# wenxiaoshuai/Points-Matching

Hardware: AMD Instinct MI355X
Metric: descriptor-pair distances/s (BF-L2 2-NN + ratio stage); RANSAC hypotheses/s in `ransac` (higher is better)
Workload: dtype f32

## Files before the change

include/pm.h:

```cpp
#ifndef PM_H_
#define PM_H_

#include <stddef.h>
#include <stdint.h>

#ifdef __cplusplus
extern "C" {
#endif

#define PM_VERSION_MAJOR 0
#define PM_VERSION_MINOR 1

typedef enum pm_status {
    PM_OK            =  0,
    PM_E_INVALID     = -1,
    PM_E_TOO_FEW     = -2,
    PM_E_NO_MODEL    = -3,
    PM_E_HIP         = -4,
    PM_E_NOMEM       = -5,
    PM_E_UNSUPPORTED = -6
} pm_status;

typedef struct pm_match {
    int32_t queryIdx;
    int32_t trainIdx;
    int32_t imgIdx;
    float   distance;
} pm_match;

typedef struct pm_ctx pm_ctx;

int  pm_ctx_create(int device, pm_ctx** out);
int  pm_ctx_destroy(pm_ctx* ctx);
int  pm_ctx_set_stream(pm_ctx* ctx, void* hip_stream);
int  pm_ctx_synchronize(pm_ctx* ctx);
int  pm_ctx_timing_enable(pm_ctx* ctx, int enable);
int  pm_ctx_timing_reset(pm_ctx* ctx);
int  pm_ctx_timing_get(pm_ctx* ctx, const char* kernel, double* mean_ms, int* launches);
int  pm_ctx_knn_diag_enable(pm_ctx* ctx, int enable);
int  pm_ctx_knn_stats(pm_ctx* ctx, int* rescans, int* nonfinite);
int  pm_ctx_knn_route(pm_ctx* ctx, int* route);
int  pm_ctx_filter_fusion_status(pm_ctx* ctx, int* gave_up);
enum {
    PM_OPT_RANSAC_PATH    = 1,
    PM_OPT_SCORE_OPERANDS = 2,
    PM_OPT_HAMMING_ROUTE  = 3,
    PM_OPT_KNN_F16_WAVES  = 4,
    PM_OPT_KNN_STAGING    = 6,
    PM_OPT_KNN_WG_PER_CU  = 7,
    PM_OPT_FILTER_FUSION  = 5,
    PM_OPT_KNN_XCD_TILE   = 8,
    PM_OPT_KNN_GENERAL_F16 = 9,
    PM_OPT_KNN_SEEDED     = 10,
    PM_OPT_KNN_U8_GROUP   = 11,
    PM_OPT_KNN_RING       = 12,
    PM_OPT_KNN_U8_REFINE  = 13,
    PM_OPT_KNN_RING_PROLOGUE = 14,
    PM_OPT_KNN_WIDE       = 15,
    PM_OPT_KNN_PREP_ROWS  = 16,
    PM_OPT_RANSAC_FORM    = 17,
    PM_OPT_RANSAC_WG_IDS  = 18,
    PM_OPT_HAMMING_REFINE = 19,
    PM_OPT_COUNT_         = 20
};
int  pm_ctx_set_option(pm_ctx* ctx, int option, int value);
int  pm_ctx_get_option(pm_ctx* ctx, int option, int* value);
const char* pm_last_error(void);
const char* pm_status_string(int status);
int  pm_version(void);

#define PM_MAX_K 16
#define PM_KNN_FORCE_EXACT  1
#define PM_KNN_FORCE_F32    2
#define PM_KNN_HINT_INTEGER 4
#define PM_KNN_HINT_U8      8
#define PM_KNN_HINT_UNIT_NORM 16
int pm_bf_knn_l2_f32(pm_ctx* ctx, const float* q, int nq, const float* t, int nt,
                     int dim, int k, int flags, pm_match* out);
int pm_bf_knn_l2_f32_dev(pm_ctx* ctx, const float* d_q, int nq, const float* d_t, int nt,
                         int dim, int k, int flags, pm_match* d_out);

int pm_bf_knn_l2_u8(pm_ctx* ctx, const uint8_t* q, int nq, const uint8_t* t, int nt, int dim, int k, pm_match* out);
int pm_bf_knn_l2_u8_dev(pm_ctx* ctx, const uint8_t* d_q, int nq, const uint8_t* d_t, int nt, int dim, int k, pm_match* d_out);
int pm_bf_knn_l2_u8_ratio_dev(pm_ctx* ctx, const uint8_t* d_q, int nq, const uint8_t* d_t, int nt, int dim, float ratio,
                              const float* d_kp1_xy, const float* d_kp2_xy, pm_match* d_knn, pm_match* d_good,
                              float* d_xy1, float* d_xy2, int32_t* d_n_good);

int pm_bf_knn_l2_ratio_dev(pm_ctx* ctx, const float* d_q, int nq, const float* d_t, int nt, int dim, int flags,
                           float ratio, const float* d_kp1_xy, const float* d_kp2_xy, pm_match* d_knn,
                           pm_match* d_good, float* d_xy1, float* d_xy2, int32_t* d_n_good);

typedef struct pm_flann_params {
    int32_t  trees;
    int32_t  checks;
    uint64_t seed;
} pm_flann_params;
typedef struct pm_flann_index pm_flann_index;
int pm_flann_build(pm_ctx* ctx, const float* train, int nt, int dim, const pm_flann_params* prm, pm_flann_index** out);
int pm_flann_destroy(pm_flann_index* ix);
int pm_flann_knn_l2_f32(pm_ctx* ctx, pm_flann_index* ix, const float* q, int nq, int k, pm_match* out);
int pm_flann_knn_l2_f32_dev(pm_ctx* ctx, pm_flann_index* ix, const float* d_q, int nq, int k, pm_match* d_out);
int pm_flann_export(const pm_flann_index* ix, int32_t* n_nodes, int32_t* roots, void* nodes, int32_t cap_nodes);

int pm_bf_knn_hamming_u8(pm_ctx* ctx, const uint8_t* q, int nq, const uint8_t* t, int nt,
                         int bytes, int k, pm_match* out);
int pm_bf_knn_hamming_u8_dev(pm_ctx* ctx, const uint8_t* d_q, int nq, const uint8_t* d_t, int nt,
                             int bytes, int k, pm_match* d_out);


int pm_filter_midpoint(const pm_match* m, int n, double* min_out, double* max_out,
                       pm_match* out, int* n_out);
int pm_filter_ratio(const pm_match* knn, int nq, int k, float ratio, pm_match* out, int* n_out);
int pm_filter_ratio_gather_dev(pm_ctx* ctx, const pm_match* d_knn, int nq, int k, float ratio,
                               const float* d_kp1_xy, const float* d_kp2_xy, pm_match* d_good,
                               float* d_xy1, float* d_xy2, int32_t* d_n_good);
int pm_filter_midpoint_gather_dev(pm_ctx* ctx, const pm_match* d_m, int n, int k,
                                  const float* d_kp1_xy, const float* d_kp2_xy, pm_match* d_good,
                                  float* d_xy1, float* d_xy2, int32_t* d_n_good, double* d_minmax);
int pm_concat_points_dev(pm_ctx* ctx, const float* d_xy1_parts, const float* d_xy2_parts,
                         const int32_t* d_counts, int parts, int stride, float* d_xy1,
                         float* d_xy2, int32_t* d_n_total);

int pm_match_indices(const pm_match* m, int n, int32_t* query_idx, int32_t* train_idx);
int pm_gather_points(const float* kp_xy, int n_kp, const int32_t* idx, int n, float* out_xy);
long pm_format_match_list(const pm_match* m, int n, char* buf, size_t cap);

enum { PM_ERR_SAMPSON = 0, PM_ERR_SYM_EPIPOLAR = 1 };

typedef struct pm_ransac_params {
    int64_t  hyp_begin;
    int64_t  hyp_end;
    uint64_t seed;
    float    thresh_px;
    int32_t  error_kind;
} pm_ransac_params;

int pm_ransac_fundamental(pm_ctx* ctx, const float* xy1, const float* xy2, int n,
                          const pm_ransac_params* p, double F[9], uint8_t* mask,
                          int* n_inliers, uint64_t* best_key);
int pm_ransac_score_dev(pm_ctx* ctx, const float* d_xy1, const float* d_xy2, int n,
                        const pm_ransac_params* p, uint64_t* d_best_key);
int pm_ransac_score_devn(pm_ctx* ctx, const float* d_xy1, const float* d_xy2, int n_max,
                         const int32_t* d_n, const pm_ransac_params* p, uint64_t* d_best_key);
int pm_ransac_run_dev(pm_ctx* ctx, const float* d_xy1, const float* d_xy2, int n_max,
                      const int32_t* d_n, const pm_ransac_params* p, uint64_t* d_best_key,
                      double* d_F, uint8_t* d_mask, int32_t* d_n_inliers);
int pm_ransac_model_from_key_dev(pm_ctx* ctx, const float* d_xy1, const float* d_xy2, int n_max,
                                 const int32_t* d_n, const pm_ransac_params* p,
                                 const uint64_t* d_key, double* d_F, uint8_t* d_mask,
                                 int32_t* d_n_inliers);
int pm_ransac_model_from_hyp(pm_ctx* ctx, const float* xy1, const float* xy2, int n,
                             const pm_ransac_params* p, int64_t hyp, double F[9],
                             uint8_t* mask, int* n_inliers);
#define PM_MAX_PARTS 64
typedef struct pm_points_view {
    const float*   xy1;
    const float*   xy2;
    const int32_t* counts;
    int32_t parts;
    int32_t cap;
    int64_t pitch_xy;
    int32_t pitch_cnt;
    int32_t reserved;
} pm_points_view;
typedef struct pm_ransac_record {
    uint64_t key;
    double   F[9];
} pm_ransac_record;
int pm_ransac_shard_parts_dev(pm_ctx* ctx, const pm_points_view* view, const pm_ransac_params* p,
                              pm_ransac_record* d_record);
int pm_ransac_finish_parts_dev(pm_ctx* ctx, const pm_points_view* view, const pm_ransac_params* p,
                               const pm_ransac_record* d_records, int n_records, uint64_t* d_key, double* d_F,
                               uint8_t* d_mask, int mask_len, int32_t* d_n_inliers, int32_t* d_n_total);
static inline uint64_t pm_ransac_key(uint32_t inliers, uint32_t hyp) {
    return ((uint64_t)inliers << 32) | (uint64_t)(0xFFFFFFFFu - hyp);
}
static inline uint32_t pm_ransac_key_hyp(uint64_t key)     { return 0xFFFFFFFFu - (uint32_t)key; }
static inline uint32_t pm_ransac_key_inliers(uint64_t key) { return (uint32_t)(key >> 32); }

enum { PM_ERR_REPROJ = 2 };
int pm_ransac_homography(pm_ctx* ctx, const float* xy1, const float* xy2, int n, const pm_ransac_params* p,
                         double H[9], uint8_t* mask, int* n_inliers, uint64_t* best_key);
int pm_ransac_homography_run_dev(pm_ctx* ctx, const pm_points_view* view, const pm_ransac_params* p,
                                 uint64_t* d_best_key, double* d_H, uint8_t* d_mask, int mask_len,
                                 int32_t* d_n_inliers);
int pm_ransac_homography_from_hyp(pm_ctx* ctx, const float* xy1, const float* xy2, int n,
                                  const pm_ransac_params* p, int64_t hyp, double H[9], uint8_t* mask,
                                  int* n_inliers);

typedef struct pm_h_refine_info {
    double  cost_in, cost_out;
    int32_t n_used, iters, status, reserved;
} pm_h_refine_info;
int pm_homography_refine(pm_ctx* ctx, const float* xy1, const float* xy2, int n, const uint8_t* mask,
                         const double H_in[9], int max_iters, double H_out[9], pm_h_refine_info* info);
int pm_homography_refine_dev(pm_ctx* ctx, const pm_points_view* view, const uint8_t* d_mask, const double* d_H_in,
                             int max_iters, double* d_H_out, pm_h_refine_info* d_info);
int pm_ransac_homography_refined(pm_ctx* ctx, const float* xy1, const float* xy2, int n, const pm_ransac_params* p,
                                 int max_iters, double H[9], uint8_t* mask, int* n_inliers, uint64_t* best_key,
                                 pm_h_refine_info* info);

enum { PM_AFFINE_FULL = 0, PM_AFFINE_PARTIAL = 1 };
int pm_ransac_affine(pm_ctx* ctx, int model, const float* xy1, const float* xy2, int n, const pm_ransac_params* p,
                     double A[6], uint8_t* mask, int* n_inliers, uint64_t* best_key);
int pm_ransac_affine_from_hyp(pm_ctx* ctx, int model, const float* xy1, const float* xy2, int n,
                              const pm_ransac_params* p, int64_t hyp, double A[6], uint8_t* mask, int* n_inliers);
int pm_ransac_affine_run_dev(pm_ctx* ctx, int model, const pm_points_view* view, const pm_ransac_params* p,
                             uint64_t* d_best_key, double* d_A, uint8_t* d_mask, int mask_len, int32_t* d_n_inliers);
int pm_affine_refine(pm_ctx* ctx, int model, const float* xy1, const float* xy2, int n, const uint8_t* mask,
                     const double A_in[6], double A_out[6], pm_h_refine_info* info);
int pm_affine_refine_dev(pm_ctx* ctx, int model, const pm_points_view* view, const uint8_t* d_mask, const double* d_A_in,
                         double* d_A_out, pm_h_refine_info* d_info);
int pm_estimate_affine(pm_ctx* ctx, int model, const float* xy1, const float* xy2, int n, const pm_ransac_params* p,
                       int refine, double A[6], uint8_t* mask, int* n_inliers, uint64_t* best_key,
                       pm_h_refine_info* info);

// ... 101 lines not shown
```

points_matching_amd/api.py:

```python
import ctypes as C
import os

import numpy as np

_HERE = os.path.dirname(os.path.abspath(__file__))
LIB_PATH = os.environ.get("PM_LIB_PATH") or os.path.join(_HERE, "libpm_hip.so")

MATCH_DTYPE = np.dtype([("queryIdx", "<i4"), ("trainIdx", "<i4"), ("imgIdx", "<i4"),
                        ("distance", "<f4")])
PM_MAX_K = 16
PM_KNN_FORCE_EXACT = 1
PM_KNN_FORCE_F32 = 2
PM_KNN_HINT_INTEGER = 4
PM_KNN_HINT_U8 = 8
PM_KNN_HINT_UNIT_NORM = 16
PM_ERR_SAMPSON = 0
PM_ERR_SYM_EPIPOLAR = 1
PM_ERR_REPROJ = 2
PM_AFFINE_FULL = 0
PM_AFFINE_PARTIAL = 1
PM_OK, PM_E_INVALID, PM_E_TOO_FEW, PM_E_NO_MODEL, PM_E_HIP, PM_E_NOMEM, PM_E_UNSUPPORTED = \
    0, -1, -2, -3, -4, -5, -6

EXPORTS = [
    "pm_ctx_create", "pm_ctx_destroy", "pm_ctx_set_stream", "pm_ctx_synchronize",
    "pm_ctx_timing_enable", "pm_ctx_timing_reset", "pm_ctx_timing_get", "pm_ctx_knn_diag_enable", "pm_ctx_knn_stats", "pm_ctx_knn_route",
    "pm_ctx_filter_fusion_status",
    "pm_last_error",
    "pm_status_string", "pm_version",
    "pm_bf_knn_l2_f32", "pm_bf_knn_l2_f32_dev", "pm_bf_knn_hamming_u8", "pm_bf_knn_hamming_u8_dev",
    "pm_filter_midpoint", "pm_filter_ratio", "pm_match_indices", "pm_gather_points",
    "pm_format_match_list",
    "pm_filter_ratio_gather_dev", "pm_filter_midpoint_gather_dev", "pm_concat_points_dev",
    "pm_ransac_fundamental", "pm_ransac_score_dev", "pm_ransac_score_devn", "pm_ransac_model_from_hyp",
    "pm_ransac_model_from_key_dev", "pm_ransac_run_dev", "pm_ransac_shard_parts_dev", "pm_ransac_finish_parts_dev",
    "pm_ctx_set_option", "pm_ctx_get_option", "pm_bf_knn_l2_ratio_dev",
    "pm_flann_build", "pm_flann_destroy", "pm_flann_knn_l2_f32", "pm_flann_knn_l2_f32_dev", "pm_flann_export",
    "pm_mgpu_create", "pm_mgpu_destroy", "pm_mgpu_size", "pm_mgpu_ctx", "pm_mgpu_ransac_fundamental", "pm_mgpu_match_ransac",
    "pm_mgpu_lane_ctx", "pm_mgpu_set_lanes", "pm_mgpu_set_train", "pm_mgpu_set_train_dev", "pm_mgpu_submit_dev", "pm_mgpu_collect",
    "pm_mgpu_allgather_latency", "pm_mgpu_batch_run", "pm_mgpu_batch_set_option",
    "pm_batch_create", "pm_batch_destroy", "pm_batch_run", "pm_batch_set_option", "pm_batch_set_desc_type", "pm_batch_set_host_threads",
    "pm_bf_knn_l2_u8", "pm_bf_knn_l2_u8_dev", "pm_bf_knn_l2_u8_ratio_dev", "pm_host_register", "pm_host_unregister",
    "pm_lmeds_fundamental", "pm_lmeds_fundamental_dev", "pm_lmeds_default_iters", "pm_ransac7_adaptive",
    "pm_epipolar_residuals", "pm_f_scale_f33", "pm_epilines", "pm_epiline_endpoints",
    "pm_ransac_homography", "pm_ransac_homography_run_dev", "pm_ransac_homography_from_hyp",
    "pm_homography_refine", "pm_homography_refine_dev", "pm_ransac_homography_refined",
    "pm_ransac_affine", "pm_ransac_affine_from_hyp", "pm_ransac_affine_run_dev", "pm_affine_refine", "pm_affine_refine_dev",
    "pm_estimate_affine",
    "pm_ransac_essential", "pm_ransac_essential_from_hyp", "pm_ransac_essential_run_dev", "pm_recover_pose",
    "pm_recover_pose_dev", "pm_estimate_pose",
]


class PmError(RuntimeError):
    def __init__(self, status, msg):
        super().__init__("pm status %d: %s" % (status, msg))
        self.status = status


class RansacParams(C.Structure):
    _fields_ = [("hyp_begin", C.c_int64), ("hyp_end", C.c_int64), ("seed", C.c_uint64),
                ("thresh_px", C.c_float), ("error_kind", C.c_int32)]


class PointsView(C.Structure):
    _fields_ = [("xy1", C.c_void_p), ("xy2", C.c_void_p), ("counts", C.c_void_p), ("parts", C.c_int32),
                ("cap", C.c_int32), ("pitch_xy", C.c_int64), ("pitch_cnt", C.c_int32), ("reserved", C.c_int32)]


class Camera(C.Structure):
    _fields_ = [("fx", C.c_double), ("fy", C.c_double), ("cx", C.c_double), ("cy", C.c_double)]


def _camera(K):
    if isinstance(K, Camera):
        return K
    k = np.asarray(K, np.float64)
    if k.shape == (3, 3):
        return Camera(k[0, 0], k[1, 1], k[0, 2], k[1, 2])
    return Camera(*[float(v) for v in k.reshape(4)])


class HRefineInfo(C.Structure):
    _fields_ = [("cost_in", C.c_double), ("cost_out", C.c_double), ("n_used", C.c_int32), ("iters", C.c_int32),
                ("status", C.c_int32), ("reserved", C.c_int32)]


H_REFINE_INFO_DTYPE = np.dtype([("cost_in", "<f8"), ("cost_out", "<f8"), ("n_used", "<i4"), ("iters", "<i4"),
                                ("status", "<i4"), ("reserved", "<i4")])

RANSAC_RECORD_DTYPE = np.dtype([("key", "<u8"), ("F", "<f8", (9,))])
PM_MAX_PARTS = 64
PM_OPT_RANSAC_PATH, PM_OPT_SCORE_OPERANDS, PM_OPT_HAMMING_ROUTE, PM_OPT_KNN_F16_WAVES, PM_OPT_FILTER_FUSION = 1, 2, 3, 4, 5
PM_OPT_KNN_STAGING = 6
PM_OPT_KNN_WG_PER_CU = 7
PM_OPT_KNN_XCD_TILE = 8
PM_OPT_KNN_GENERAL_F16 = 9
PM_OPT_KNN_SEEDED = 10
PM_OPT_KNN_U8_GROUP = 11
PM_OPT_KNN_RING = 12
PM_OPT_KNN_U8_REFINE = 13
PM_OPT_KNN_RING_PROLOGUE = 14
PM_OPT_KNN_WIDE = 15
PM_OPT_KNN_PREP_ROWS = 16
PM_OPT_RANSAC_FORM = 17
PM_OPT_RANSAC_WG_IDS = 18
PM_OPT_HAMMING_REFINE = 19


_lib = None


def lib():
    global _lib
    if _lib is None:
        if not os.path.exists(LIB_PATH):
            raise PmError(PM_E_UNSUPPORTED,
                          "%s is missing: run `python -m points_matching_amd.build`" % LIB_PATH)
        try:
            import torch
        except ImportError:
            pass
        _lib = C.CDLL(LIB_PATH)
        _lib.pm_last_error.restype = C.c_char_p
        _lib.pm_status_string.restype = C.c_char_p
        _lib.pm_format_match_list.restype = C.c_long
    return _lib


def _check(rc):
    if rc != PM_OK:
        raise PmError(rc, (lib().pm_last_error() or b"").decode() or
                      lib().pm_status_string(rc).decode())


def _p(a):
    return a.ctypes.data_as(C.c_void_p) if a is not None else None


def _pair(xy1, xy2):
    xy1 = np.ascontiguousarray(xy1, np.float32).reshape(-1, 2)
    xy2 = np.ascontiguousarray(xy2, np.float32).reshape(-1, 2)
    if xy2.shape[0] != xy1.shape[0]:
        raise ValueError("xy1 and xy2 must have the same length")
    return xy1, xy2, xy1.shape[0]


def _outcome(rc):
    if rc not in (PM_OK, PM_E_NO_MODEL, PM_E_TOO_FEW):
        _check(rc)
    return rc


def ransac_key(inliers, hyp):
    return (int(inliers) << 32) | (0xFFFFFFFF - int(hyp))


def ransac_key_hyp(key):
    return 0xFFFFFFFF - (int(key) & 0xFFFFFFFF)


def ransac_key_inliers(key):
    return int(key) >> 32



def filter_midpoint(m):
    m = np.ascontiguousarray(m, MATCH_DTYPE).reshape(-1)
    out = np.zeros(max(m.size, 1), MATCH_DTYPE)
    mn, mx, n = C.c_double(), C.c_double(), C.c_int()
    _check(lib().pm_filter_midpoint(_p(m), m.size, C.byref(mn), C.byref(mx), _p(out), C.byref(n)))
    return out[:n.value].copy(), mn.value, mx.value


def filter_ratio(knn, ratio):
    knn = np.ascontiguousarray(knn, MATCH_DTYPE)
    nq, k = knn.shape
    out = np.zeros(max(nq, 1), MATCH_DTYPE)
    n = C.c_int()
    _check(lib().pm_filter_ratio(_p(knn), nq, k, C.c_float(ratio), _p(out), C.byref(n)))
    return out[:n.value].copy()


def match_indices(m):
    m = np.ascontiguousarray(m, MATCH_DTYPE).reshape(-1)
    qi = np.zeros(m.size, np.int32)
    ti = np.zeros(m.size, np.int32)
    _check(lib().pm_match_indices(_p(m), m.size, _p(qi), _p(ti)))
    return qi, ti


def gather_points(kp_xy, idx):
    kp_xy = np.ascontiguousarray(kp_xy, np.float32).reshape(-1, 2)
    idx = np.ascontiguousarray(idx, np.int32)
    out = np.zeros((idx.size, 2), np.float32)
    _check(lib().pm_gather_points(_p(kp_xy), kp_xy.shape[0], _p(idx), idx.size, _p(out)))
    return out


def format_match_list(m):
    m = np.ascontiguousarray(m, MATCH_DTYPE).reshape(-1)
    need = lib().pm_format_match_list(_p(m), m.size, None, C.c_size_t(0))
    buf = C.create_string_buffer(need + 1)
    lib().pm_format_match_list(_p(m), m.size, buf, C.c_size_t(need + 1))
    return buf.value.decode()


def epipolar_residuals(xy1, xy2, F, transposed=1):
    xy1 = np.ascontiguousarray(xy1, np.float32)
    xy2 = np.ascontiguousarray(xy2, np.float32)
    F = np.ascontiguousarray(F, np.float64).reshape(9)
    n = xy1.shape[0]
    r = np.zeros(max(n, 1), np.float64)
    mean = C.c_double()
    _check(lib().pm_epipolar_residuals(_p(xy1), _p(xy2), n, _p(F), transposed, _p(r), C.byref(mean)))
    return r[:n], mean.value


def f_scale_f33(F):
    F = np.ascontiguousarray(F, np.float64).reshape(9).copy()
    _check(lib().pm_f_scale_f33(_p(F)))
    return F.reshape(3, 3)


def epilines(xy, which_image, F):
    xy = np.ascontiguousarray(xy, np.float32)
    F = np.ascontiguousarray(F, np.float64).reshape(9)
    lines = np.zeros((xy.shape[0], 3), np.float32)
    _check(lib().pm_epilines(_p(xy), xy.shape[0], which_image, _p(F), _p(lines)))
    return lines


def epiline_endpoints(lines, cols):
    lines = np.ascontiguousarray(lines, np.float32)
    out = np.zeros((lines.shape[0], 4), np.int32)
    _check(lib().pm_epiline_endpoints(_p(lines), lines.shape[0], cols, _p(out)))
    return out



class Context:

    def __init__(self, device=0):
        self._h = C.c_void_p()
        _check(lib().pm_ctx_create(device, C.byref(self._h)))

    def close(self):
        if self._h:
            lib().pm_ctx_destroy(self._h)
            self._h = C.c_void_p()

    def __del__(self):
        try:
            self.close()
        except Exception:
            pass

    def __enter__(self):
        return self

# ... 614 lines not shown
```

points_matching_amd/csrc/knn_coarse.hip:

```cpp
#include "knn_coarse_kernels.hpp"

namespace pm_knn {

int launch_coarse_f32(pm_ctx* ctx, const float* dq, int nq, const float* dt, int nt, int dim, const float* tnorm,
                      int splits, int tiles_per_split, unsigned keep_mask, float* cval, int slots,
                      const unsigned long long* stats, unsigned epoch, int only_if_ineligible)
{
    return coarse_f32_dispatch<AblNone>(ctx, dq, nq, dt, nt, dim, tnorm, splits, tiles_per_split, keep_mask, cval, slots,
                                        stats, epoch, only_if_ineligible);
}

int launch_coarse_f16(pm_ctx* ctx, const _Float16* Qh, const _Float16* Th, int nq, int nq_pad, int nt, int splits,
                      int tiles_per_split, unsigned keep_mask, float* cval, int slots,
                      const unsigned long long* stats, unsigned epoch, int mode, int dp)
{
    if (dp == 256)
        return launch_rows288<RouteF16T<256>, AblNone>(ctx, "knn_l2_mfma_f16", Qh, Th, nullptr, nq, nq_pad, nt, splits, tiles_per_split,
                                                  keep_mask, cval, slots, stats, epoch, mode);
    return launch_rows288<RouteF16, AblNone>(ctx, "knn_l2_mfma_f16", Qh, Th, nullptr, nq, nq_pad, nt, splits, tiles_per_split, keep_mask,
                                        cval, slots, stats, epoch, mode);
}

int launch_coarse_i8(pm_ctx* ctx, const void* Qe, const void* Te, int nq, int nq_pad, int nt, int splits,
                     int tiles_per_split, int* cval, int slots)
{
    return launch_rows288<RouteI8, AblNone>(ctx, "knn_hamming_mfma_i8", Qe, Te, nullptr, nq, nq_pad, nt, splits, tiles_per_split, 0u,
                                   cval, slots, nullptr, 0u, 0);
}

int launch_coarse_u8(pm_ctx* ctx, const void* Q8, const void* T8, const int* seeds, int nq, int nq_pad, int nt, int splits,
                     int tiles_per_split, int* cval, int slots, int group_rows, int form)
{
    return coarse_u8_dispatch<AblNone>(ctx, Q8, T8, seeds, nq, nq_pad, nt, splits, tiles_per_split, cval, slots, group_rows, form);
}

int launch_coarse_f16s(pm_ctx* ctx, const _Float16* Qh, const _Float16* Th, const float* seeds, int nq, int nq_pad, int nt,
                       int splits, int tiles_per_split, unsigned keep_mask, float* cval, int slots)
{
    return launch_rows288<RouteF16S, AblNone>(ctx, "knn_l2_mfma_f16s", Qh, Th, seeds, nq, nq_pad, nt, splits, tiles_per_split,
                                         keep_mask, cval, slots, nullptr, 0u, 0);
}

}
```

points_matching_amd/csrc/knn_coarse_kernels.hpp:

```cpp
#pragma once
#include <type_traits>

#include "knn_shared.hpp"

namespace pm_knn {
namespace {

template <bool NO_EPI, bool NO_STAGE, bool NO_BARRIER, bool NO_LDSREAD>
struct Abl {
    static constexpr bool no_epi = NO_EPI;
    static constexpr bool no_stage = NO_STAGE;
    static constexpr bool no_barrier = NO_BARRIER;
    static constexpr bool no_ldsread = NO_LDSREAD;
    static __device__ __forceinline__ void stamp(int) {}
};
typedef Abl<false, false, false, false> AblNone;

struct WgTile { int qb, split; };
__device__ __forceinline__ WgTile wg_tile(bool tiled)
{
    const int nx = gridDim.x, ny = gridDim.y;
    if (!tiled || (nx & 3) || (ny & 1)) return WgTile{static_cast<int>(blockIdx.x), static_cast<int>(blockIdx.y)};
    const int L = blockIdx.y * nx + blockIdx.x;
    const int x = L & 7, j = L >> 3;
// ... 366 lines not shown
#pragma unroll
        for (int i = 0; i < PIECES; ++i) {
            int f = tid + THREADS * i;
            if (!EVEN) f = f < TOTAL ? f : TOTAL - 1;
            stg[i] = Th[static_cast<size_t>(tile) * TOTAL + f];
        }
    }
    __device__ __forceinline__ void store(uint4* __restrict__ hsm, int buf, int tid) const
    {
#pragma unroll
        for (int i = 0; i < PIECES; ++i) {
            const int f = tid + THREADS * i;
            const int row = f / R::ROW16, c8 = f % R::ROW16;
            if (EVEN || f < TOTAL) hsm[(buf * H_TT + row) * R::LDS_ROW16 + c8] = stg[i];
        }
    }
};

template <typename R, int THREADS>
struct HTileDma {
    static constexpr int NW = THREADS / 64;
    static constexpr int SLOTS = H_TT * R::LDS_ROW16;
    static_assert(SLOTS % 64 == 0, "the padded tile must be a whole number of 1-KiB pieces");
    static constexpr int NPIECES = SLOTS / 64;
    static constexpr int PER_WAVE = (NPIECES + NW - 1) / NW;
    static constexpr int TOTAL = H_TT * R::ROW16;
    unsigned src[PER_WAVE];
    __device__ __forceinline__ void init(int lane, int wave)
    {
#pragma unroll
        for (int i = 0; i < PER_WAVE; ++i) {
            const int p = wave + NW * i;
            const int s = 64 * (p < NPIECES ? p : NPIECES - 1) + lane;
            const int row = s / R::LDS_ROW16, c = s % R::LDS_ROW16;
            src[i] = static_cast<unsigned>(row * R::ROW16 + (c < R::ROW16 ? c : R::ROW16 - 1));
        }
    }
    __device__ __forceinline__ void issue(__amdgpu_buffer_rsrc_t rsrc, int tile, uint4* __restrict__ hsm, int buf, int wave) const
    {
        typedef __attribute__((address_space(3))) void* lptr_t;
        const int soff = tile * (TOTAL * 16);
#pragma unroll
        for (int i = 0; i < PER_WAVE; ++i) {
            const int p = wave + NW * i;
            if (p < NPIECES) {
                uint4* l = hsm + buf * SLOTS + 64 * p;
                __builtin_amdgcn_raw_ptr_buffer_load_lds(rsrc, (lptr_t)l, 16, static_cast<int>(src[i]) * 16, soff, 0, 0);
            }
        }
    }
};

struct Seed64 { uint4 v[4]; };
template <typename R, int NQB, bool EPI, typename ABL>
__device__ __forceinline__ void h_block(const uint4* __restrict__ tb, const uint4* __restrict__ sb,
                                        const typename R::frag (&qf)[NQB][R::NCH],
                                        typename R::acc (&a)[NQB], const typename R::acc (&p)[NQB], unsigned pbase,
                                        unsigned par, typename R::list (&cl)[NQB])
{
    typedef typename R::frag frag;
    typename R::acc seed = R::zero();
    if constexpr (R::SEEDED) seed = __builtin_bit_cast(typename R::acc, Seed64{{sb[0], sb[1], sb[2], sb[3]}});
    frag ring[3];
#pragma unroll
    for (int c = 0; c < 3; ++c) ring[c] = *reinterpret_cast<const frag*>(tb + 2 * c);
#pragma unroll
    for (int c = 0; c < R::NCH; ++c) {
        const frag x = ring[c % 3];
        if constexpr (!ABL::no_ldsread) {
            if (c + 3 < R::NCH) ring[c % 3] = *reinterpret_cast<const frag*>(tb + 2 * (c + 3));
        }
#pragma unroll
        for (int qb = 0; qb < NQB; ++qb) a[qb] = R::mfma(x, qf[qb][c], c == 0 ? seed : a[qb]);
        if constexpr (ABL::no_epi) {
            if (EPI && c == 1) {
#pragma unroll
                for (int qb = 0; qb < NQB; ++qb)
#pragma unroll
                    for (int e = 0; e < 16; ++e) asm volatile("" ::"v"(p[qb][e]));
            }
        }
        if (EPI && c >= 1 && !ABL::no_epi) {
            constexpr int NGB = R::GPB * NQB;
#pragma unroll
            for (int e = (c - 1) * NGB / (R::NCH - 1); e < c * NGB / (R::NCH - 1); ++e)
                R::select(p[e % NQB], par, (pbase + static_cast<unsigned>(e / NQB)) << 1, cl[e % NQB], e / NQB);
            if (NQB == 2)
                asm volatile("" : "+v"(cl[0][0]), "+v"(cl[0][1]), "+v"(cl[0][2]), "+v"(cl[0][3]), "+v"(cl[NQB - 1][0]),
                             "+v"(cl[NQB - 1][1]), "+v"(cl[NQB - 1][2]), "+v"(cl[NQB - 1][3]));
            else
                asm volatile("" : "+v"(cl[0][0]), "+v"(cl[0][1]), "+v"(cl[0][2]), "+v"(cl[0][3]));
        }
    }
}

template <typename R, int NQB, bool FIRST, typename ABL>
__device__ __forceinline__ void h_tile(const uint4* __restrict__ tb, const uint4* __restrict__ sb,
                                       const typename R::frag (&qf)[NQB][R::NCH], typename R::acc (&A)[NQB],
                                       typename R::acc (&B)[NQB], unsigned lb, unsigned par, typename R::list (&cl)[NQB])
{
    typedef typename R::frag frag;
    typedef typename R::acc acc;
    constexpr int NCH = R::NCH, STEPS = 4 * NCH, PF = 3;
    constexpr unsigned G = R::GPB;
    auto a_ptr = [&](int step) { return reinterpret_cast<const frag*>(tb + (step / NCH) * 32 * R::LDS_ROW16 + 2 * (step % NCH)); };
    auto seed_of = [&](int blk) {
        if constexpr (R::SEEDED) {
            const uint4* p = sb + 8 * blk;
            return __builtin_bit_cast(acc, Seed64{{p[0], p[1], p[2], p[3]}});
        } else {
            return R::zero();
        }
    };
    frag ring[PF];
#pragma unroll
    for (int i = 0; i < PF; ++i) ring[i] = *a_ptr(i);
    acc seed = seed_of(0);
#pragma unroll
    for (int s_ = 0; s_ < STEPS; ++s_) {
        const int blk = s_ / NCH, c = s_ % NCH;
        const frag x = ring[s_ % PF];
        if constexpr (!ABL::no_ldsread) {
            if (s_ + PF < STEPS) ring[s_ % PF] = *a_ptr(s_ + PF);
        }
        acc(&cur)[NQB] = (blk & 1) ? B : A;
        const acc(&prev)[NQB] = (blk & 1) ? A : B;
#pragma unroll
        for (int qb = 0; qb < NQB; ++qb) cur[qb] = R::mfma(x, qf[qb][c], c == 0 ? seed : cur[qb]);
        if (c == 0 && blk < 3) seed = seed_of(blk + 1);
        const bool epi = !(FIRST && blk == 0);
        if constexpr (ABL::no_epi) {
            if (epi && c == 1) {
#pragma unroll
                for (int qb = 0; qb < NQB; ++qb)
#pragma unroll
                    for (int e = 0; e < 16; ++e) asm volatile("" ::"v"(prev[qb][e]));
            }
        }
        if (epi && c >= 1 && !ABL::no_epi) {
            constexpr int NGB = R::GPB * NQB;
            const unsigned pbase = lb + G * static_cast<unsigned>(blk) - G;
#pragma unroll
            for (int e = (c - 1) * NGB / (NCH - 1); e < c * NGB / (NCH - 1); ++e)
                R::select(prev[e % NQB], par, (pbase + static_cast<unsigned>(e / NQB)) << 1, cl[e % NQB], e / NQB);
            if (NQB == 2)
                asm volatile("" : "+v"(cl[0][0]), "+v"(cl[0][1]), "+v"(cl[0][2]), "+v"(cl[0][3]), "+v"(cl[NQB - 1][0]),
                             "+v"(cl[NQB - 1][1]), "+v"(cl[NQB - 1][2]), "+v"(cl[NQB - 1][3]));
            else
                asm volatile("" : "+v"(cl[0][0]), "+v"(cl[0][1]), "+v"(cl[0][2]), "+v"(cl[0][3]));
        }
    }
}

template <typename R, int NQB, bool DMA, int GR, typename ABL>
__global__ __launch_bounds__(H_QB / (32 * NQB) * 64 * GR, (R::NCH > 9 ? (NQB == 2 ? 1 : 2) : (NQB == 2 ? 2 : 4))) void knn_mfma_rows288(
    const uint4* __restrict__ Qh, const uint4* __restrict__ Th, const uint4* __restrict__ seeds_g, int nq, int nt,
    int tiles_per_split, unsigned par, typename R::list* __restrict__ cand_val, int slots,
    const unsigned long long* __restrict__ stats, unsigned epoch, int mode)
{
    typedef typename R::frag frag;
    typedef typename R::acc acc;
    typedef typename R::list list;
    constexpr int WPG = H_QB / (32 * NQB);
    constexpr int THREADS = WPG * 64 * GR;
    static_assert(GR == 1 || (GR == 2 && NQB == 2 && R::MERGE), "row groups: the 64-query form of a merged-list route");
    if (mode & 1) {
        const unsigned long long s1 = stats[1], s3 = stats[3];
        if (static_cast<unsigned>(s1 >> 32) == epoch && (s1 & 2ull) && static_cast<unsigned>(s3 >> 32) == epoch)
            return;
    }
    extern __shared__ __attribute__((aligned(16))) uint4 hsm[];
    static_assert(!R::SEEDED || DMA, "the seeded routes stage by LDS-DMA only");
    constexpr int TILE_SLOTS = H_TT * R::LDS_ROW16;
    uint4* const ssm = hsm + 2 * TILE_SLOTS;
    const int tid = threadIdx.x, lane = tid & 63, wave = tid >> 6;
    const int r = lane & 31, h = lane >> 5;
    const int gw = wave % WPG, grp = wave / WPG;
    const WgTile wg = wg_tile((mode & 2) != 0);
    const int qbase = wg.qb * H_QB + gw * 32 * NQB;

    HTile<R, THREADS> st;
    HTileDma<R, THREADS> dma;
    const int ntiles = (nt + H_TT - 1) / H_TT;
    const int tile0 = wg.split * tiles_per_split;
    const __amdgpu_buffer_rsrc_t t_rsrc = __builtin_amdgcn_make_buffer_rsrc(
        const_cast<uint4*>(Th), 0, ntiles * (H_TT * R::ROW16 * 16), 0x00020000);
    const __amdgpu_buffer_rsrc_t s_rsrc = __builtin_amdgcn_make_buffer_rsrc(
        const_cast<uint4*>(R::SEEDED ? seeds_g : Th), 0, (ntiles + 1) * SEED_TILE_BYTES, 0x00020000);
    auto seed_issue = [&](int tile, int buf) {
        typedef __attribute__((address_space(3))) void* lptr_t;
        if (R::SEEDED && wave == THREADS / 64 - 1)
            __builtin_amdgcn_raw_ptr_buffer_load_lds(s_rsrc, (lptr_t)(ssm + 64 * buf), 16, lane * 16, tile * SEED_TILE_BYTES, 0, 0);
    };
    if (DMA) {
        dma.init(lane, wave);
        dma.issue(t_rsrc, tile0 < ntiles ? tile0 : ntiles - 1, hsm, 0, wave);
        seed_issue(tile0 < ntiles ? tile0 : ntiles - 1, 0);
    } else {
        st.load(Th, tile0 < ntiles ? tile0 : ntiles - 1, tid);
    }
    frag qf[NQB][R::NCH];
#pragma unroll
    for (int qb = 0; qb < NQB; ++qb)
#pragma unroll
        for (int c = 0; c < R::NCH; ++c)
            qf[qb][c] = *reinterpret_cast<const frag*>(Qh + static_cast<size_t>(qbase + 32 * qb + r) * R::ROW16 + 2 * c + h);
#pragma unroll
    for (int qb = 0; qb < NQB; ++qb)
#pragma unroll
        for (int c = 0; c < R::NCH; ++c) {
            typedef unsigned u32x4 __attribute__((ext_vector_type(4)));
            u32x4 t = __builtin_bit_cast(u32x4, qf[qb][c]);
            asm volatile("" : "+v"(t));
            qf[qb][c] = __builtin_bit_cast(frag, t);
        }

    int tile1 = tile0 + tiles_per_split;
    if (tile1 > ntiles) tile1 = ntiles;
    list cl[NQB];
#pragma unroll
    for (int qb = 0; qb < NQB; ++qb) cl[qb] = R::empty();

    if (tile0 < tile1) {
        if (!DMA) st.store(hsm, 0, tid);
        __syncthreads();
        acc A[NQB], B[NQB];
        for (int tix = 0; tix < tile1 - tile0; ++tix) {
            const int buf = tix & 1;
            const uint4* tb = hsm + (buf * H_TT + r) * R::LDS_ROW16 + h;
            constexpr unsigned G = R::GPB;
            const unsigned lb = static_cast<unsigned>(tix) * (4u * G);
            if constexpr (!ABL::no_stage) {
                if (DMA) {
                    dma.issue(t_rsrc, tile0 + tix + 1 < ntiles ? tile0 + tix + 1 : tile0 + tix, hsm, buf ^ 1, wave);
                    seed_issue(tile0 + tix + 1 < ntiles ? tile0 + tix + 1 : tile0 + tix, buf ^ 1);
                } else st.load(Th, tile0 + tix + 1 < ntiles ? tile0 + tix + 1 : tile0 + tix, tid);
            }
            const uint4* sb = ssm + 64 * buf + 4 * h;
            if constexpr (GR == 1) {
                if (tix == 0) h_block<R, NQB, false, ABL>(tb, sb, qf, A, A, 0u, par, cl);
                else h_block<R, NQB, true, ABL>(tb, sb, qf, A, B, lb - G, par, cl);
                h_block<R, NQB, true, ABL>(tb + 32 * R::LDS_ROW16, sb + 8, qf, B, A, lb, par, cl);
                h_block<R, NQB, true, ABL>(tb + 64 * R::LDS_ROW16, sb + 16, qf, A, B, lb + G, par, cl);
                if constexpr (!ABL::no_stage) {
                    if (!DMA) st.store(hsm, buf ^ 1, tid);
                }
                h_block<R, NQB, true, ABL>(tb + 96 * R::LDS_ROW16, sb + 24, qf, B, A, lb + 2u * G, par, cl);
            } else {
                const uint4* tg = tb + grp * 64 * R::LDS_ROW16;
                const uint4* sg = sb + 16 * grp;
                const unsigned gb = lb + 2u * static_cast<unsigned>(grp) * G;
                if (tix == 0) h_block<R, NQB, false, ABL>(tg, sg, qf, A, A, 0u, par, cl);
                else h_block<R, NQB, true, ABL>(tg, sg, qf, A, B, gb - 3u * G, par, cl);
                if constexpr (!ABL::no_stage) {
                    if (!DMA) st.store(hsm, buf ^ 1, tid);
                }
                h_block<R, NQB, true, ABL>(tg + 32 * R::LDS_ROW16, sg + 8, qf, B, A, gb, par, cl);
            }
            tile_barrier<ABL>();
        }
        const unsigned lb = static_cast<unsigned>(tile1 - tile0 - 1) * (4u * R::GPB) +
                            (GR == 1 ? 3u : 2u * static_cast<unsigned>(grp) + 1u) * R::GPB;
#pragma unroll
        for (int qb = 0; qb < NQB; ++qb)
#pragma unroll
            for (int g = 0; g < R::GPB; ++g) R::select(B[qb], par, (lb + static_cast<unsigned>(g)) << 1, cl[qb], g);
    }
    if constexpr (GR == 2) {
        list* xs = reinterpret_cast<list*>(hsm);
#pragma unroll
        for (int qb = 0; qb < NQB; ++qb) {
            R::merge(cl[qb], h);
            if (grp == 1) xs[(gw * NQB + qb) * 64 + lane] = cl[qb];
        }
        __syncthreads();
        if (grp == 1) return;
#pragma unroll
        for (int qb = 0; qb < NQB; ++qb) {
            const list o = xs[(gw * NQB + qb) * 64 + lane];
#pragma unroll
            for (int i = 0; i < 4; ++i) R::put(cl[qb], o[i]);
            const int q = qbase + 32 * qb + r;
            if (q < nq && h == 0) cand_val[(static_cast<size_t>(q) * slots + wg.split * KNN_C) / KNN_C] = cl[qb];
        }
        return;
    }
#pragma unroll
    for (int qb = 0; qb < NQB; ++qb) {
        const int q = qbase + 32 * qb + r;
        R::merge(cl[qb], h);
        if (R::MERGE) {
            if (q < nq && h == 0) cand_val[(static_cast<size_t>(q) * slots + wg.split * KNN_C) / KNN_C] = cl[qb];
        } else {
            if (q < nq) cand_val[(static_cast<size_t>(q) * slots + (wg.split * 2 + h) * KNN_C) / KNN_C] = cl[qb];
        }
    }
}

template <int N>
__device__ __forceinline__ void wait_vmcnt_imm() { asm volatile("s_waitcnt vmcnt(%0)" ::"n"(N) : "memory"); }
template <int BASE>
__device__ __forceinline__ void wait_tiles(int ahead, bool plus)
{
    static_assert(7 * (BASE + 1) <= 63, "vmcnt is a 6-bit counter");
#define PM_W(A_) case A_: if (plus) wait_vmcnt_imm<A_ * (BASE + 1)>(); else wait_vmcnt_imm<A_ * BASE>(); break;
    switch (ahead) {
        PM_W(1) PM_W(2) PM_W(3) PM_W(4) PM_W(5) PM_W(6) PM_W(7)
        default: wait_vmcnt_imm<0>(); break;
    }
#undef PM_W
}

template <typename FRAG>
__device__ __forceinline__ FRAG untracked_load16(const void* p)
{
    typedef unsigned u32x4 __attribute__((ext_vector_type(4)));
    u32x4 v;
    asm volatile("global_load_dwordx4 %0, %1, off" : "=&v"(v) : "v"(p) : "memory");
    return __builtin_bit_cast(FRAG, v);
}
template <typename FRAG>
__device__ __forceinline__ void pin_after_wait(FRAG& f)
{
    typedef unsigned u32x4 __attribute__((ext_vector_type(4)));
    u32x4 t = __builtin_bit_cast(u32x4, f);
    asm volatile("" : "+v"(t)::"memory");
    f = __builtin_bit_cast(FRAG, t);
}

template <typename R, int NQB, int WAVES, int NBUF, bool SPLIT, typename ABL>
__global__ __launch_bounds__(WAVES * 64, WAVES / 4) void knn_mfma_ring(
    const uint4* __restrict__ Qh, const uint4* __restrict__ Th, const uint4* __restrict__ seeds_g, int nq, int nt,
    int tiles_per_split, unsigned par, typename R::list* __restrict__ cand_val, int slots, int mode, int pro)
{
    typedef typename R::frag frag;
    typedef typename R::acc acc;
    typedef typename R::list list;
    constexpr int THREADS = WAVES * 64;
    constexpr int QB_WG = WAVES * 32 * NQB;
    constexpr int TILE_SLOTS = H_TT * R::LDS_ROW16;
    typedef HTileDma<R, THREADS> Dma;
    static_assert(NBUF >= 3 && NBUF <= 8, "ring of three to eight buffers (wait_tiles covers up to 7 tiles in flight)");
    extern __shared__ __attribute__((aligned(16))) uint4 hsm[];
    uint4* const ssm = hsm + NBUF * TILE_SLOTS;
    int* const arrive = reinterpret_cast<int*>(ssm + NBUF * 64);
    int* const done = arrive + NBUF;
    const int tid = threadIdx.x, lane = tid & 63, wave = tid >> 6;
    const int r = lane & 31, h = lane >> 5;
    const WgTile wg = wg_tile((mode & 2) != 0);
    const int qbase = wg.qb * QB_WG + wave * 32 * NQB;
    ABL::stamp(0);
    if constexpr (SPLIT) {
        if (tid < 2 * NBUF) arrive[tid] = 0;
        asm volatile("s_waitcnt lgkmcnt(0)" ::: "memory");
        __builtin_amdgcn_s_barrier();
        asm volatile("" ::: "memory");
    }
    auto poll = [&](int* ctr, int target) {
        for (;;) {
            const int v = __builtin_amdgcn_readfirstlane(__hip_atomic_load(ctr, __ATOMIC_RELAXED, __HIP_MEMORY_SCOPE_WORKGROUP));
            if (v >= target) break;
            __builtin_amdgcn_s_sleep(1);
        }
        asm volatile("" ::: "memory");
    };
    auto bump = [&](int* ctr) {
        if (lane == 0) __hip_atomic_fetch_add(ctr, 1, __ATOMIC_RELAXED, __HIP_MEMORY_SCOPE_WORKGROUP);
    };

    const int ntiles = (nt + H_TT - 1) / H_TT;
    const int tile0 = wg.split * tiles_per_split;
    int tile1 = tile0 + tiles_per_split;
    if (tile1 > ntiles) tile1 = ntiles;
    const int ntl = tile1 - tile0;

    frag qf[NQB][R::NCH];
#pragma unroll
    for (int qb = 0; qb < NQB; ++qb)
#pragma unroll
        for (int c = 0; c < R::NCH; ++c)
            qf[qb][c] = untracked_load16<frag>(Qh + static_cast<size_t>(qbase + 32 * qb + r) * R::ROW16 + 2 * c + h);

    const __amdgpu_buffer_rsrc_t t_rsrc = __builtin_amdgcn_make_buffer_rsrc(
        const_cast<uint4*>(Th), 0, ntiles * (H_TT * R::ROW16 * 16), 0x00020000);
    const __amdgpu_buffer_rsrc_t s_rsrc = __builtin_amdgcn_make_buffer_rsrc(
        const_cast<uint4*>(R::SEEDED ? seeds_g : Th), 0, (ntiles + 1) * SEED_TILE_BYTES, 0x00020000);
    Dma dma;
    dma.init(lane, wave);
    constexpr int BASE = Dma::NPIECES / Dma::NW;
    const int own = (Dma::NPIECES - wave + Dma::NW - 1) / Dma::NW + ((R::SEEDED && wave == Dma::NW - 1) ? 1 : 0);
    const bool plus = __builtin_amdgcn_readfirstlane(own) != BASE;
    static_assert(Dma::NPIECES >= Dma::NW, "every wave issues at least one piece");
    auto request = [&](int t) {
        typedef __attribute__((address_space(3))) void* lptr_t;
        const int buf = t % NBUF;
        dma.issue(t_rsrc, tile0 + t, hsm, buf, wave);
        if (R::SEEDED && wave == Dma::NW - 1)
            __builtin_amdgcn_raw_ptr_buffer_load_lds(s_rsrc, (lptr_t)(ssm + 64 * buf), 16, lane * 16, (tile0 + t) * SEED_TILE_BYTES, 0, 0);
    };
    int next = 0;
    auto pump = [&](int done_below, int most) {
        for (int n = 0; n < most && next < ntl && next < done_below + NBUF; ++n) {
            if constexpr (SPLIT) {
                if (next >= NBUF) poll(&done[next % NBUF], WAVES * (next / NBUF));
            }
            request(next);
            ++next;
        }
    };
    pump(0, pro);
    if constexpr (SPLIT) {
        if (ntl > 0) {
            asm volatile("s_waitcnt vmcnt(0)" ::: "memory");
            bump(&arrive[0]);
        }
    }
    ABL::stamp(1);

    list cl[NQB];
#pragma unroll
    for (int qb = 0; qb < NQB; ++qb) cl[qb] = R::empty();

    if (ntl > 0) {
        acc A[NQB], B[NQB];
        constexpr unsigned G = R::GPB;
#pragma unroll 1
        for (int tix = 0; tix < ntl; ++tix) {
            if constexpr (SPLIT) {
                if constexpr (!ABL::no_barrier) poll(&arrive[tix % NBUF], WAVES * (tix / NBUF + 1));
                if constexpr (!ABL::no_stage) pump(tix, 2);
                if (tix + 1 < ntl) {
                    wait_tiles<BASE>(next - 2 - tix, plus);
                    bump(&arrive[(tix + 1) % NBUF]);
                }
            } else {
                if (tix == 0) asm volatile("s_waitcnt vmcnt(0)" ::: "memory");
                else wait_tiles<BASE>(next - 1 - tix, plus);
                if constexpr (!ABL::no_barrier) __builtin_amdgcn_s_barrier();
                asm volatile("" ::: "memory");
            }
#pragma unroll
            for (int qb = 0; qb < NQB; ++qb)
#pragma unroll
                for (int c = 0; c < R::NCH; ++c) pin_after_wait(qf[qb][c]);
            __builtin_amdgcn_sched_barrier(0);
            if constexpr (!SPLIT && !ABL::no_stage) pump(tix, 2);
            if (tix < 14) ABL::stamp(2 + tix);
            const int buf = tix % NBUF;
            const uint4* tb = hsm + (buf * H_TT + r) * R::LDS_ROW16 + h;
            const uint4* sb = ssm + 64 * buf + 4 * h;
            const unsigned lb = static_cast<unsigned>(tix) * (4u * G);
            if (tix == 0) h_tile<R, NQB, true, ABL>(tb, sb, qf, A, B, lb, par, cl);
            else h_tile<R, NQB, false, ABL>(tb, sb, qf, A, B, lb, par, cl);
            if constexpr (SPLIT) {
                if (tix + NBUF < ntl) bump(&done[tix % NBUF]);
            }
        }
        const unsigned lb = static_cast<unsigned>(ntl - 1) * (4u * G) + 3u * G;
#pragma unroll
        for (int qb = 0; qb < NQB; ++qb)
#pragma unroll
            for (int g = 0; g < R::GPB; ++g) R::select(B[qb], par, (lb + static_cast<unsigned>(g)) << 1, cl[qb], g);
    }
    ABL::stamp(16);
#pragma unroll
    for (int qb = 0; qb < NQB; ++qb) {
        const int q = qbase + 32 * qb + r;
        R::merge(cl[qb], h);
        if (R::MERGE) {
            if (q < nq && h == 0) cand_val[(static_cast<size_t>(q) * slots + wg.split * KNN_C) / KNN_C] = cl[qb];
        } else {
            if (q < nq) cand_val[(static_cast<size_t>(q) * slots + (wg.split * 2 + h) * KNN_C) / KNN_C] = cl[qb];
        }
    }
    ABL::stamp(17);
}

template <typename R>
inline bool rows288_dma_ok(int nt) { return (static_cast<long long>(nt) + H_TT) * (R::ROW16 * 16) < 0x7FFFFFFFLL; }

inline bool xcd_tiled(const pm_ctx* ctx) { return ctx->opts[PM_OPT_KNN_XCD_TILE] != 1; }

template <int NCH, bool FULL, int TT, typename ABL>
int launch_mfma(pm_ctx* ctx, const float* dq, int nq, const float* dt, int nt, int dim, const float* tnorm, int splits,
                int tiles_per_split, unsigned keep_mask, float* cval, int slots, const unsigned long long* stats,
                unsigned epoch, int only_if_ineligible)
{
    constexpr int LDT = NCH * 8 + 4;
    const size_t lds = 2 * TT * LDT * sizeof(float);
    static bool attr_done_dev[PM_MAX_DEVICES] = {};
    bool& attr_done = attr_done_dev[ctx->device];
    if (!attr_done) {
        PM_HIP_CHECK(hipFuncSetAttribute(reinterpret_cast<const void*>(&knn_l2_mfma<NCH, FULL, TT, ABL>),
                                         hipFuncAttributeMaxDynamicSharedMemorySize, static_cast<int>(lds)));
        attr_done = true;
    }
    dim3 grid((nq + QB - 1) / QB, splits);
    const int mode = (only_if_ineligible ? 1 : 0) | (xcd_tiled(ctx) ? 2 : 0);
    pm::ScopedKernelTime t(ctx, "knn_l2_mfma");
    hipLaunchKernelGGL((knn_l2_mfma<NCH, FULL, TT, ABL>), grid, dim3(256), lds, ctx->stream, dq, dt, tnorm, nq, nt, dim,
                       tiles_per_split, keep_mask, cval, slots, stats, epoch, mode);
    PM_HIP_CHECK(hipGetLastError());
    return PM_OK;
}

template <typename ABL>
int coarse_f32_dispatch(pm_ctx* ctx, const float* dq, int nq, const float* dt, int nt, int dim, const float* tnorm,
                      int splits, int tiles_per_split, unsigned keep_mask, float* cval, int slots,
                      const unsigned long long* stats, unsigned epoch, int only_if_ineligible)
{
#define PM_LAUNCH_MFMA(NCH_, FULL_)                                                                              \
    launch_mfma<NCH_, FULL_, TT32, ABL>(ctx, dq, nq, dt, nt, dim, tnorm, splits, tiles_per_split, keep_mask, cval, slots, \
                                   stats, epoch, only_if_ineligible)
    if (dim == 128) return PM_LAUNCH_MFMA(16, true);
    if (dim == 64) return PM_LAUNCH_MFMA(8, true);
    if (dim == 32) return PM_LAUNCH_MFMA(4, true);
    if (dim < 32) return PM_LAUNCH_MFMA(4, false);
    if (dim < 64) return PM_LAUNCH_MFMA(8, false);
    return PM_LAUNCH_MFMA(16, false);
#undef PM_LAUNCH_MFMA
}

template <typename R, typename ABL>
int launch_rows288(pm_ctx* ctx, const char* name, const void* Qh, const void* Th, const void* seeds, int nq, int nq_pad, int nt,
                   int splits, int tiles_per_split, unsigned par, void* cval, int slots, const unsigned long long* stats,
                   unsigned epoch, int mode)
{
    const size_t lds = sizeof(uint4) * (2 * H_TT * R::LDS_ROW16 + (R::SEEDED ? 2 * 64 : 0));
    const int nqb_opt = ctx->opts[PM_OPT_KNN_F16_WAVES];
    const int nqb = nqb_opt ? nqb_opt : (tiles_per_split <= 8 ? 1 : 2);
    static bool attr_done_dev[PM_MAX_DEVICES] = {};
    bool& attr_done = attr_done_dev[ctx->device];
    if (!attr_done) {
#define PM_ATTR(NQB_, DMA_, GR_)                                                                                  \
    PM_HIP_CHECK(hipFuncSetAttribute(reinterpret_cast<const void*>(&knn_mfma_rows288<R, NQB_, DMA_, GR_, ABL>),        \
                                     hipFuncAttributeMaxDynamicSharedMemorySize, static_cast<int>(lds)))
        PM_ATTR(1, true, 1); PM_ATTR(2, true, 1);
        if constexpr (!R::SEEDED) { PM_ATTR(1, false, 1); PM_ATTR(2, false, 1); }
        if constexpr (R::MERGE) {
            PM_ATTR(2, true, 2);
            if constexpr (!R::SEEDED) PM_ATTR(2, false, 2);
        }
#undef PM_ATTR
        attr_done = true;
    }
    pm::ScopedKernelTime t(ctx, name);
    const uint4* q4 = static_cast<const uint4*>(Qh);
    const uint4* t4 = static_cast<const uint4*>(Th);
    const uint4* s4 = static_cast<const uint4*>(seeds);
    typename R::list* out = static_cast<typename R::list*>(cval);
    const bool dma = R::SEEDED || (ctx->opts[PM_OPT_KNN_STAGING] != 1 && rows288_dma_ok<R>(nt));
    PM_REQUIRE(!R::SEEDED || rows288_dma_ok<R>(nt), PM_E_UNSUPPORTED, "train set too large for the seeded coarse routes");
#define PM_GO(NQB_, DMA_, GR_, THREADS_)                                                                           \
    hipLaunchKernelGGL((knn_mfma_rows288<R, NQB_, DMA_, GR_, ABL>), dim3(nq_pad / H_QB, splits), dim3(THREADS_), lds,  \
                       ctx->stream, q4, t4, s4, nq, nt, tiles_per_split, par, out, slots, stats, epoch, mode)
#define PM_GO2(NQB_, GR_, THREADS_)                                                                                \
    do {                                                                                                           \
        if constexpr (R::SEEDED) { PM_GO(NQB_, true, GR_, THREADS_); }                                             \
        else { if (dma) PM_GO(NQB_, true, GR_, THREADS_); else PM_GO(NQB_, false, GR_, THREADS_); }                \
    } while (0)
    mode = (mode ? 1 : 0) | (xcd_tiled(ctx) ? 2 : 0);
    bool grouped = false;
    if constexpr (R::MERGE) {
        if (nqb == 3) {
            grouped = true;
            PM_GO2(2, 2, 512);
        }
    }
    if (grouped) { }
    else if (nqb == 2) PM_GO2(2, 1, 256);
    else PM_GO2(1, 1, 512);
#undef PM_GO2
#undef PM_GO
    PM_HIP_CHECK(hipGetLastError());
    return PM_OK;
}

inline int ring_qb_wg(const pm_ctx* ctx) { return ctx->opts[PM_OPT_KNN_F16_WAVES] == 3 ? 512 : 256; }
template <typename R, int NBUF, typename ABL>
int launch_ring(pm_ctx* ctx, const char* name, const void* Qh, const void* Th, const void* seeds, int nq, int nq_pad, int nt,
                int splits, int tiles_per_split, unsigned par, void* cval, int slots)
{
    const size_t lds = static_cast<size_t>(NBUF) * (sizeof(uint4) * H_TT * R::LDS_ROW16 + 1024) + 64;
    static_assert(static_cast<size_t>(NBUF) * (sizeof(uint4) * H_TT * R::LDS_ROW16 + 1024) + 64 <= 160 * 1024, "ring exceeds the CU's LDS");
    const bool split = ctx->opts[PM_OPT_KNN_RING] == 3;
    PM_REQUIRE(rows288_dma_ok<R>(nt), PM_E_UNSUPPORTED, "train set too large for the LDS-DMA coarse routes");
    const int form = ctx->opts[PM_OPT_KNN_F16_WAVES];
    const int qb_wg = ring_qb_wg(ctx);
    PM_REQUIRE(nq_pad % qb_wg == 0, PM_E_INVALID, "query padding does not match the workgroup size");
    static bool attr_done_dev[PM_MAX_DEVICES] = {};
    bool& attr_done = attr_done_dev[ctx->device];
    if (!attr_done) {
#define PM_ATTR(NQB_, WAVES_)                                                                                        \
    PM_HIP_CHECK(hipFuncSetAttribute(reinterpret_cast<const void*>(&knn_mfma_ring<R, NQB_, WAVES_, NBUF, false, ABL>),    \
                                     hipFuncAttributeMaxDynamicSharedMemorySize, static_cast<int>(lds)));                \
    PM_HIP_CHECK(hipFuncSetAttribute(reinterpret_cast<const void*>(&knn_mfma_ring<R, NQB_, WAVES_, NBUF, true, ABL>),     \
                                     hipFuncAttributeMaxDynamicSharedMemorySize, static_cast<int>(lds)))
        PM_ATTR(1, 8); PM_ATTR(2, 4); PM_ATTR(1, 16);
#undef PM_ATTR
        attr_done = true;
    }
    pm::ScopedKernelTime t(ctx, name);
    const uint4* q4 = static_cast<const uint4*>(Qh);
    const uint4* t4 = static_cast<const uint4*>(Th);
    const uint4* s4 = static_cast<const uint4*>(seeds);
    typename R::list* out = static_cast<typename R::list*>(cval);
    const int mode = xcd_tiled(ctx) ? 2 : 0;
    int pro = ctx->opts[PM_OPT_KNN_RING_PROLOGUE] ? ctx->opts[PM_OPT_KNN_RING_PROLOGUE] : 2;
    if (pro < 2) pro = 2;
#define PM_GO1(NQB_, WAVES_, SPLIT_)                                                                                \
    hipLaunchKernelGGL((knn_mfma_ring<R, NQB_, WAVES_, NBUF, SPLIT_, ABL>), dim3(nq_pad / qb_wg, splits), dim3(WAVES_ * 64), lds, \
                       ctx->stream, q4, t4, s4, nq, nt, tiles_per_split, par, out, slots, mode, pro)
#define PM_GO(NQB_, WAVES_) do { if (split) PM_GO1(NQB_, WAVES_, true); else PM_GO1(NQB_, WAVES_, false); } while (0)
    if (form == 3) PM_GO(1, 16);
    else if (form == 2) PM_GO(2, 4);
    else PM_GO(1, 8);
#undef PM_GO
#undef PM_GO1
    PM_HIP_CHECK(hipGetLastError());
    return PM_OK;
}

constexpr int RA_NQB = 4;
constexpr int RA_WAVES = 8;
constexpr int RA_QB = 32 * RA_NQB;

constexpr int RA_PIECES = 5;
constexpr int RA_PRIV_SLOTS = RA_PIECES * 64;

template <int GPB_, bool PRIV, bool WSPLIT, typename ABL>
__global__ __launch_bounds__(RA_WAVES * 64, 1) void knn_u8_rega(const uint4* __restrict__ Q8, const uint4* __restrict__ T8,
                                                               const uint4* __restrict__ seeds_g, int nq, int nt, int tiles_per_split,
                                                               i32x4* __restrict__ cand_val, int slots, int mode)
{
    typedef RouteU8T<GPB_> R;
    typedef typename R::frag frag;
    typedef typename R::acc acc;
    typedef typename R::list list;
    __shared__ list xs[RA_WAVES][RA_NQB][64];
    extern __shared__ __attribute__((aligned(16))) uint4 psm[];
    const int tid = threadIdx.x, lane = tid & 63, wave = __builtin_amdgcn_readfirstlane(tid >> 6);
    const int r = lane & 31, h = lane >> 5;
    const WgTile wg = wg_tile((mode & 2) != 0);
    const int qbase = WSPLIT ? wg.qb * (2 * RA_QB) + (wave >> 2) * RA_QB : wg.qb * RA_QB;

    const int ntiles = (nt + H_TT - 1) / H_TT;
    const int my_split = WSPLIT ? wg.split * (RA_WAVES / 2) + (wave & 3) : wg.split;
    const int tile0 = my_split * tiles_per_split;
    int tile1 = tile0 + tiles_per_split;
    if (tile1 > ntiles) tile1 = ntiles;
    const int nblocks = tile1 > tile0 ? (tile1 - tile0) * 4 : 0;
    const int block0 = tile0 * 4;
    constexpr int STEP = WSPLIT ? 1 : RA_WAVES;
    if (WSPLIT && nblocks == 0) return;

    struct Ops { frag a[U8_NCH]; Seed64 s; };
    constexpr int T_ROW_BYTES = (PRIV ? U8_WIDE_ROW16 : U8_ROW16) * 16;
    int src[RA_PIECES];
#pragma unroll
    for (int p = 0; p < RA_PIECES; ++p) {
        const int sl = 64 * p + lane, row = sl / U8_LDS_ROW16, u = sl % U8_LDS_ROW16;
        (void)row; (void)u;
        src[p] = (sl < 32 * U8_LDS_ROW16 ? sl : 32 * U8_LDS_ROW16 - 1) * 16;
    }
    const __amdgpu_buffer_rsrc_t t_rsrc = __builtin_amdgcn_make_buffer_rsrc(
        const_cast<uint4*>(T8), 0, ntiles * (H_TT * T_ROW_BYTES), 0x00020000);
    uint4* const mine = psm + wave * (3 * RA_PRIV_SLOTS);
    auto load_ops = [&](int blk, Ops& o, int buf) {
        if constexpr (PRIV) {
            typedef __attribute__((address_space(3))) void* lptr_t;
            const int soff = (block0 + blk) * (32 * T_ROW_BYTES);
#pragma unroll
            for (int p = 0; p < RA_PIECES; ++p)
                __builtin_amdgcn_raw_ptr_buffer_load_lds(t_rsrc, (lptr_t)(mine + buf * RA_PRIV_SLOTS + 64 * p), 16, src[p], soff, 0, 0);
        } else {
            const uint4* tp = T8 + (static_cast<size_t>(block0 + blk) * 32 + r) * U8_ROW16 + h;
#pragma unroll
            for (int c = 0; c < U8_NCH; ++c) o.a[c] = *reinterpret_cast<const frag*>(tp + 2 * c);
        }
        const uint4* sp = seeds_g + static_cast<size_t>(block0 + blk) * 8 + 4 * h;
#pragma unroll
        for (int i = 0; i < 4; ++i) {
            if constexpr (PRIV) { }
            else o.s.v[i] = sp[i];
        }
    };
    constexpr int OPS_PER_BLOCK = RA_PIECES;
    ABL::stamp(0);
    Ops o0, o1;
    int b = WSPLIT ? 0 : wave;
    if (!PRIV && b < nblocks) load_ops(b, o0, 0);
    frag qf[RA_NQB][U8_NCH];
#pragma unroll
    for (int qb = 0; qb < RA_NQB; ++qb)
#pragma unroll
        for (int c = 0; c < U8_NCH; ++c)
            qf[qb][c] = *reinterpret_cast<const frag*>(Q8 + static_cast<size_t>(qbase + 32 * qb + r) * U8_ROW16 + 2 * c + h);
    if constexpr (PRIV) asm volatile("s_waitcnt vmcnt(0)" ::: "memory");
#pragma unroll
    for (int qb = 0; qb < RA_NQB; ++qb)
#pragma unroll
        for (int c = 0; c < U8_NCH; ++c) {
            typedef unsigned u32x4 __attribute__((ext_vector_type(4)));
            u32x4 t = __builtin_bit_cast(u32x4, qf[qb][c]);
            asm volatile("" : "+v"(t));
            qf[qb][c] = __builtin_bit_cast(frag, t);
        }
    list cl[RA_NQB];
#pragma unroll
    for (int qb = 0; qb < RA_NQB; ++qb) cl[qb] = R::empty();
    ABL::stamp(1);
    if (PRIV && !WSPLIT && b < nblocks) load_ops(b, o0, 0);

    auto block = [&](Ops& o, int blk, int buf) {
        const int sk = blk / STEP - 4;
        if (sk >= 0 && sk < 3) ABL::stamp(2 + 4 * sk);
        if constexpr (PRIV) {
            asm volatile("s_waitcnt vmcnt(%0)" ::"n"(2 * OPS_PER_BLOCK) : "memory");
            {
                const uint4* sq = mine + buf * RA_PRIV_SLOTS + 4 * h * U8_LDS_ROW16 + U8_ROW16;
#pragma unroll
                for (int i = 0; i < 4; ++i) o.s.v[i] = sq[i * U8_LDS_ROW16];
            }
            const uint4* tb = mine + buf * RA_PRIV_SLOTS + r * U8_LDS_ROW16 + h;
#pragma unroll
            for (int c = 0; c < U8_NCH; ++c) o.a[c] = *reinterpret_cast<const frag*>(tb + 2 * c);
// ... 55 lines not shown
#pragma unroll
            for (int c = 0; c < U8_NCH; ++c) a[c] = *reinterpret_cast<const frag*>(base + r * U8_LDS_ROW16 + h + 2 * c);
            if (sk >= 0 && sk < 3) ABL::stamp(3 + 4 * sk);
            const acc seed = __builtin_bit_cast(acc, sd);
            const unsigned gb = static_cast<unsigned>(blk - 1) * R::GPB;
            constexpr int NGB = R::GPB * RA_NQB;
#pragma unroll
            for (int c = 0; c < U8_NCH; ++c) {
#pragma unroll
                for (int qb = 0; qb < RA_NQB; ++qb) cur[qb] = R::mfma(a[c], qf[qb][c], c == 0 ? seed : cur[qb]);
                if constexpr (decltype(has_prev)::value) {
                    if (c >= 1) {
                        if constexpr (ABL::no_epi) {
                            if (c == 1) {
#pragma unroll
                                for (int qb = 0; qb < RA_NQB; ++qb)
#pragma unroll
                                    for (int e = 0; e < 16; ++e) asm volatile("" ::"v"(prev[qb][e]));
                            }
                        } else {
#pragma unroll
                            for (int e = (c - 1) * NGB / (U8_NCH - 1); e < c * NGB / (U8_NCH - 1); ++e)
                                R::select(prev[e % RA_NQB], 0u, (gb + static_cast<unsigned>(e / RA_NQB)) << 1, cl[e % RA_NQB], e / RA_NQB);
                            asm volatile("" : "+v"(cl[0][0]), "+v"(cl[1][0]), "+v"(cl[2][0]), "+v"(cl[3][0]));
                        }
                    }
                }
            }
            if (sk >= 0 && sk < 3) { ABL::stamp(4 + 4 * sk); ABL::stamp(5 + 4 * sk); }
        };
        const int last = nblocks - 1;
        int bc = 0, bn = 2;
        issue(0, 0);
        issue(1 < last ? 1 : last, 1);
        b = 0;
        issue(2 < last ? 2 : last, 2);
        wblock(0, 0, accA, accB, std::false_type{});
        b = 1; bc = 1; bn = 0;
        while (true) {
            if (b >= nblocks) break;
            issue(b + 2 < last ? b + 2 : last, bn);
            wblock(bc, b, accB, accA, std::true_type{});
            ++b; bc = bc == 2 ? 0 : bc + 1; bn = bn == 2 ? 0 : bn + 1;
            if (b >= nblocks) break;
            issue(b + 2 < last ? b + 2 : last, bn);
            wblock(bc, b, accA, accB, std::true_type{});
            ++b; bc = bc == 2 ? 0 : bc + 1; bn = bn == 2 ? 0 : bn + 1;
        }
        if constexpr (!ABL::no_epi) {
            if (((nblocks - 1) & 1) == 0) select_all(accA, nblocks - 1);
            else select_all(accB, nblocks - 1);
        }
    } else if constexpr (PRIV) {
        const int last = nblocks > 0 ? b + (nblocks - 1 - b) / STEP * STEP : 0;
        Ops o2;
        if (b < nblocks) {
            load_ops(b + STEP < last ? b + STEP : last, o1, 1);
            while (true) {
                load_ops(b + 2 * STEP < last ? b + 2 * STEP : last, o2, 2);
                block(o0, b, 0);
                b += STEP;
                if (b >= nblocks) break;
                load_ops(b + 2 * STEP < last ? b + 2 * STEP : last, o0, 0);
                block(o1, b, 1);
                b += STEP;
                if (b >= nblocks) break;
                load_ops(b + 2 * STEP < last ? b + 2 * STEP : last, o1, 1);
                block(o2, b, 2);
                b += STEP;
                if (b >= nblocks) break;
            }
        }
    } else {
    while (b < nblocks) {
        const int b1 = b + STEP;
        load_ops(b1 < nblocks ? b1 : b, o1, 1);
        block(o0, b, 0);
        if (b1 >= nblocks) break;
        const int b2 = b1 + STEP;
        load_ops(b2 < nblocks ? b2 : b1, o0, 0);
        block(o1, b1, 1);
        b = b2;
    }
    }
    if constexpr (PRIV) asm volatile("s_waitcnt vmcnt(0)" ::: "memory");
    ABL::stamp(16);

    if constexpr (WSPLIT) {
#pragma unroll
        for (int qb = 0; qb < RA_NQB; ++qb) {
            R::merge(cl[qb], h);
            const int q = qbase + 32 * qb + r;
            if (q < nq && h == 0) cand_val[(static_cast<size_t>(q) * slots + my_split * KNN_C) / KNN_C] = cl[qb];
        }
        ABL::stamp(17);
        return;
    }
#pragma unroll
    for (int qb = 0; qb < RA_NQB; ++qb) {
        R::merge(cl[qb], h);
        xs[wave][qb][lane] = cl[qb];
    }
    __syncthreads();
    if (wave >= RA_NQB) return;
    list out = xs[0][wave][lane];
#pragma unroll
    for (int w = 1; w < RA_WAVES; ++w) {
        const list o = xs[w][wave][lane];
#pragma unroll
        for (int i = 0; i < 4; ++i) R::put(out, o[i]);
    }
    const int q = qbase + 32 * wave + r;
    if (q < nq && h == 0) cand_val[(static_cast<size_t>(q) * slots + wg.split * KNN_C) / KNN_C] = out;
}

template <int GPB_, typename ABL>
int launch_rega(pm_ctx* ctx, const char* name, const void* Q8, const void* T8, const void* seeds, int nq, int nq_pad, int nt,
                int splits, int tiles_per_split, void* cval, int slots, int form)
{
    PM_REQUIRE(nq_pad % RA_QB == 0, PM_E_INVALID, "query padding does not match the workgroup size");
    pm::ScopedKernelTime t(ctx, name);
    const int mode = xcd_tiled(ctx) ? 2 : 0;
    const uint4* q4 = static_cast<const uint4*>(Q8);
    const uint4* t4 = static_cast<const uint4*>(T8);
    const uint4* s4 = static_cast<const uint4*>(seeds);
    i32x4* out = static_cast<i32x4*>(cval);
    if (form >= 5) {
        PM_REQUIRE(rows288_dma_ok<RouteU8T<GPB_>>(nt) && (static_cast<long long>(nt) + 2 * H_TT) * (U8_WIDE_ROW16 * 16) < 0x7FFFFFFFLL,
                   PM_E_UNSUPPORTED, "train set too large for the LDS-DMA coarse routes");
        const size_t lds = sizeof(uint4) * RA_WAVES * 3 * RA_PRIV_SLOTS;
        static bool attr_done_dev[PM_MAX_DEVICES] = {};
        if (!attr_done_dev[ctx->device]) {
            PM_HIP_CHECK(hipFuncSetAttribute(reinterpret_cast<const void*>(&knn_u8_rega<GPB_, true, false, ABL>),
                                             hipFuncAttributeMaxDynamicSharedMemorySize, static_cast<int>(lds)));
            PM_HIP_CHECK(hipFuncSetAttribute(reinterpret_cast<const void*>(&knn_u8_rega<GPB_, true, true, ABL>),
                                             hipFuncAttributeMaxDynamicSharedMemorySize, static_cast<int>(lds)));
            attr_done_dev[ctx->device] = true;
        }
        if (form == 6)
            hipLaunchKernelGGL((knn_u8_rega<GPB_, true, true, ABL>), dim3(nq_pad / (2 * RA_QB), (splits + RA_WAVES / 2 - 1) / (RA_WAVES / 2)),
                               dim3(RA_WAVES * 64), lds, ctx->stream, q4, t4, s4, nq, nt, tiles_per_split, out, slots, mode);
        else
            hipLaunchKernelGGL((knn_u8_rega<GPB_, true, false, ABL>), dim3(nq_pad / RA_QB, splits), dim3(RA_WAVES * 64), lds,
                               ctx->stream, q4, t4, s4, nq, nt, tiles_per_split, out, slots, mode);
    } else {
        hipLaunchKernelGGL((knn_u8_rega<GPB_, false, false, ABL>), dim3(nq_pad / RA_QB, splits), dim3(RA_WAVES * 64), 0, ctx->stream,
                           q4, t4, s4, nq, nt, tiles_per_split, out, slots, mode);
    }
    PM_HIP_CHECK(hipGetLastError());
    return PM_OK;
}

template <typename ABL>
int coarse_u8_dispatch(pm_ctx* ctx, const void* Q8, const void* T8, const int* seeds, int nq, int nq_pad, int nt, int splits,
                       int tiles_per_split, int* cval, int slots, int group_rows, int form)
{
    if (form >= 4 && group_rows == 8)
        return launch_rega<2, ABL>(ctx, "knn_l2_mfma_u8", Q8, T8, seeds, nq, nq_pad, nt, splits, tiles_per_split, cval, slots, form);
    if (form >= 2 && group_rows == 8)
        return launch_ring<RouteU8T<2>, 8, ABL>(ctx, "knn_l2_mfma_u8", Q8, T8, seeds, nq, nq_pad, nt, splits, tiles_per_split, 0u, cval, slots);
#define PM_U8(GPB_)                                                                                                        \
    launch_rows288<RouteU8T<GPB_>, ABL>(ctx, "knn_l2_mfma_u8", Q8, T8, seeds, nq, nq_pad, nt, splits, tiles_per_split, 0u, cval,   \
                                        slots, nullptr, 0u, 0)
    if (group_rows == 16) return PM_U8(1);
    if (group_rows == 8) return PM_U8(2);
    return PM_U8(4);
#undef PM_U8
}

}
}
```

points_matching_amd/csrc/knn_l2.hip:

```cpp
#include <cstdlib>

#include "knn_shared.hpp"

namespace {

using namespace pm_knn;

constexpr int TILE_T = 64;
constexpr int PM_U8_FUSED_MAX_NQ = 768;
__host__ inline bool u8_fused_by_default(int nq) { return nq <= PM_U8_FUSED_MAX_NQ; }
constexpr float KNN_INF = __builtin_inff();

__device__ __forceinline__ uint32_t f32_bits(float f) { return __float_as_uint(f); }

__device__ __forceinline__ uint64_t knn_key(float dist, int idx)
{
    uint32_t b = (dist != dist) ? 0x7FC00000u : f32_bits(dist);
    return (static_cast<uint64_t>(b) << 32) | static_cast<uint32_t>(idx);
}

template <bool VEC4>
__device__ __forceinline__ float l2sqr_canonical(const float* __restrict__ a,
                                                 const float* __restrict__ b, int dim)
{
// ... 76 lines not shown
    for (int o = 32; o > 0; o >>= 1) {
        mx = max(mx, static_cast<unsigned>(__shfl_xor(static_cast<int>(mx), o, 64)));
        bad |= static_cast<unsigned>(__shfl_xor(static_cast<int>(bad), o, 64));
    }
    if ((threadIdx.x & 63) == 0) { wmax[threadIdx.x >> 6] = mx; wbad[threadIdx.x >> 6] = bad; }
    __syncthreads();
    if (threadIdx.x == 0) {
        mx = max(max(wmax[0], wmax[1]), max(wmax[2], wmax[3]));
        bad = wbad[0] | wbad[1] | wbad[2] | wbad[3];
        const unsigned long long tag = static_cast<unsigned long long>(epoch) << 32;
        if (is_t) atomicMax(&stats[0], tag | mx);
        if (bad) atomicMax(&stats[1], tag | 1ull);
    }
}

template <int DP>
struct F16Rows {
    static constexpr int ROWH = DP + 16;
    static constexpr int NCB = DP / 128;
    static constexpr float MAXABS = DP == 128 ? 361.f : 255.f;
};

template <bool ALIGNED>
struct Row8 {
    f32x4 a, b;
    float e[8];
    __device__ __forceinline__ void load(const float* __restrict__ p, int c, int dim)
    {
        if constexpr (ALIGNED) {
            const int c1 = c < dim ? c : dim - 4, c2 = c + 4 < dim ? c + 4 : dim - 4;
            a = *reinterpret_cast<const f32x4*>(p + c1);
            b = *reinterpret_cast<const f32x4*>(p + c2);
        } else {
#pragma unroll
            for (int k = 0; k < 8; ++k) e[k] = p[c + k < dim ? c + k : dim - 1];
        }
    }
    __device__ __forceinline__ void get(int c, int dim, bool live, float (&v)[8]) const
    {
#pragma unroll
        for (int k = 0; k < 8; ++k) {
            float x = ALIGNED ? (k < 4 ? a[k & 3] : b[k & 3]) : e[k];
            const bool in = ALIGNED ? (c + (k & ~3) < dim) : (c + k < dim);
            v[k] = (live && in) ? x : 0.f;
        }
    }
};

template <bool SEEDED, int DP, bool ALIGNED>
__global__ __launch_bounds__(256) void knn_l2_prep16(const float* __restrict__ Q, int nq, int nq_pad,
                                                     const float* __restrict__ T, int nt, int nt_pad, int dim,
                                                     float* __restrict__ qnorm, float* __restrict__ tnorm,
                                                     _Float16* __restrict__ Qh, _Float16* __restrict__ Th,
                                                     float* __restrict__ seeds,
                                                     unsigned long long* __restrict__ stats, unsigned epoch)
{
    typedef F16Rows<DP> G;
    constexpr int ROWH = SEEDED ? DP : G::ROWH;
    constexpr int NCB = G::NCB;
    __shared__ unsigned wmax[4];
    __shared__ unsigned wbad[4];
    const int sub = threadIdx.x & 15, grp = threadIdx.x >> 4;
    const int qblocks = nq_pad / 64;
    const bool is_t = static_cast<int>(blockIdx.x) >= qblocks;
    const float* x = is_t ? T : Q;
    const int n = is_t ? nt : nq;
    float* norm = is_t ? tnorm : qnorm;
    _Float16* xh = is_t ? Th : Qh;
    const int row0 = (is_t ? blockIdx.x - qblocks : blockIdx.x) * 64;
    unsigned mx = 0u, bad = 0u;
    const int c0 = 8 * sub;
    Row8<ALIGNED> ld[4][NCB];
#pragma unroll
    for (int it = 0; it < 4; ++it) {
        const int row = row0 + it * 16 + grp;
        const float* p = x + static_cast<size_t>(row < n ? row : n - 1) * dim;
#pragma unroll
        for (int cb = 0; cb < NCB; ++cb) ld[it][cb].load(p, 128 * cb + c0, dim);
    }
#pragma unroll
    for (int it = 0; it < 4; ++it) {
        const int row = row0 + it * 16 + grp;
        const bool live = row < n;
        float s = 0.f;
        bool okrow = true;
#pragma unroll
        for (int cb = 0; cb < NCB; ++cb) {
            float v[8];
            ld[it][cb].get(128 * cb + c0, dim, live, v);
            f16x8 hv;
#pragma unroll
            for (int e = 0; e < 8; ++e) {
                s = fmaf(v[e], v[e], s);
                okrow &= (v[e] == __builtin_rintf(v[e])) && (__builtin_fabsf(v[e]) <= G::MAXABS);
                hv[e] = static_cast<_Float16>(v[e]);
            }
            *reinterpret_cast<f16x8*>(xh + static_cast<size_t>(row) * ROWH + 128 * cb + c0) = hv;
        }
#pragma unroll
        for (int o = 8; o > 0; o >>= 1) s += __shfl_xor(s, o, 16);
        if (!okrow) bad |= 2u;
        if (sub == 0) {
            if (live) {
                norm[row] = s;
                if (!(s < KNN_INF)) bad |= 3u;
                else if (is_t) mx = max(mx, f32_bits(s));
            }
            if constexpr (SEEDED) {
                if (is_t) seeds[seed_pos(row)] = live ? -0.5f * s : -1.0e30f;
                continue;
            }
            f16x8 e0 = {0, 0, 0, 0, 0, 0, 0, 0};
            const f16x8 e1 = {0, 0, 0, 0, 0, 0, 0, 0};
            if (is_t) {
                if (live) {
                    const unsigned tn = s < 16777216.f ? static_cast<unsigned>(s) : 0u;
                    e0[0] = static_cast<_Float16>(static_cast<float>(tn >> 13));
                    e0[1] = static_cast<_Float16>(static_cast<float>((tn >> 6) & 127u));
                    e0[2] = static_cast<_Float16>(static_cast<float>(tn & 63u));
                } else {
                    e0[0] = static_cast<_Float16>(60000.f);
                }
            } else {
                e0[0] = static_cast<_Float16>(-4096.f);
                e0[1] = static_cast<_Float16>(-32.f);
                e0[2] = static_cast<_Float16>(-0.5f);
            }
            *reinterpret_cast<f16x8*>(xh + static_cast<size_t>(row) * G::ROWH + DP) = e0;
            *reinterpret_cast<f16x8*>(xh + static_cast<size_t>(row) * G::ROWH + DP + 8) = e1;
        }
    }
#pragma unroll
    for (int o = 32; o > 0; o >>= 1) {
        mx = max(mx, static_cast<unsigned>(__shfl_xor(static_cast<int>(mx), o, 64)));
        bad |= static_cast<unsigned>(__shfl_xor(static_cast<int>(bad), o, 64));
    }
    if ((threadIdx.x & 63) == 0) { wmax[threadIdx.x >> 6] = mx; wbad[threadIdx.x >> 6] = bad; }
    __syncthreads();
    if (threadIdx.x == 0) {
        mx = max(max(wmax[0], wmax[1]), max(wmax[2], wmax[3]));
        bad = wbad[0] | wbad[1] | wbad[2] | wbad[3];
        const unsigned long long tag = static_cast<unsigned long long>(epoch) << 32;
        if (is_t) atomicMax(&stats[0], tag | mx);
        if (bad) atomicMax(&stats[1], tag | static_cast<unsigned long long>(bad == 1u ? 3u : bad));
    }
}

template <int ITERS>
__global__ __launch_bounds__(256) void knn_l2_prep8(const float* __restrict__ Q, int nq, int nq_pad,
                                                    const float* __restrict__ T, int nt, int nt_pad, int dim,
                                                    float* __restrict__ qnorm, float* __restrict__ tnorm,
                                                    uint2* __restrict__ Q8, uint2* __restrict__ T8,
                                                    int* __restrict__ seeds, unsigned long long* __restrict__ stats,
                                                    unsigned epoch, int t_wide)
{
    __shared__ unsigned wbad[4];
    const int sub = threadIdx.x & 15, grp = threadIdx.x >> 4;
    const int qblocks = nq_pad / (16 * ITERS);
    const bool is_t = static_cast<int>(blockIdx.x) >= qblocks;
    const float* x = is_t ? T : Q;
    const int n = is_t ? nt : nq;
    uint2* x8 = is_t ? T8 : Q8;
    const int row0 = (is_t ? blockIdx.x - qblocks : blockIdx.x) * (16 * ITERS);
    unsigned bad = 0u;
    const int c0 = 8 * sub;
    f32x4 ld[ITERS][2];
#pragma unroll
    for (int it = 0; it < ITERS; ++it) {
        const int row = row0 + it * 16 + grp;
        const float* p = x + static_cast<size_t>(row < n ? row : n - 1) * dim;
#pragma unroll
        for (int e = 0; e < 2; ++e) {
            const int c = c0 + 4 * e < dim ? c0 + 4 * e : dim - 4;
            ld[it][e] = *reinterpret_cast<const f32x4*>(p + c);
        }
    }
#pragma unroll
    for (int it = 0; it < ITERS; ++it) {
        const int row = row0 + it * 16 + grp;
        const bool live = row < n;
        float s = 0.f;
        bool okrow = true;
        unsigned w[2] = {0u, 0u};
#pragma unroll
        for (int e = 0; e < 8; ++e) {
            const bool col = live && c0 + (e & ~3) < dim;
            const float v = ld[it][e >> 2][e & 3];
            okrow &= !col || ((v == __builtin_rintf(v)) && v >= 0.f && v <= 255.f);
            const float vc = __builtin_fminf(__builtin_fmaxf(v, 0.f), 255.f);
            const float c = col ? vc - 128.f : 0.f;
            s = fmaf(c, c, s);
            const unsigned b = col ? (static_cast<unsigned>(static_cast<int>(vc)) ^ 0x80u) : 0u;
            w[e >> 2] |= b << (8 * (e & 3));
        }
#pragma unroll
        for (int o = 8; o > 0; o >>= 1) s += __shfl_xor(s, o, 16);
        if (!okrow) bad |= 2u;
        x8[static_cast<size_t>(row) * ((is_t && t_wide) ? U8_WIDE_ROW16 * 2 : U8_DP / 8) + sub] = uint2{w[0], w[1]};
        if (sub == 0) {
            const int si = static_cast<int>(s);
            if (is_t) {
                seeds[seed_pos(row)] = live ? -(si >> 1) : U8_PAD_SEED;
                if (t_wide) reinterpret_cast<int*>(T8)[u8_wide_seed_index(row)] = live ? -(si >> 1) : U8_PAD_SEED;
                if (live) tnorm[row] = s;
            } else if (live) {
                qnorm[row] = s;
            }
        }
    }
#pragma unroll
    for (int o = 32; o > 0; o >>= 1) bad |= static_cast<unsigned>(__shfl_xor(static_cast<int>(bad), o, 64));
    if ((threadIdx.x & 63) == 0) wbad[threadIdx.x >> 6] = bad;
    __syncthreads();
    if (threadIdx.x == 0) {
        bad = wbad[0] | wbad[1] | wbad[2] | wbad[3];
        if (bad) atomicMax(&stats[1], (static_cast<unsigned long long>(epoch) << 32) | 3ull);
    }
}

__global__ __launch_bounds__(256) void knn_l2_prep8_u8(const uint8_t* __restrict__ Q, int nq, int nq_pad,
                                                       const uint8_t* __restrict__ T, int nt, int nt_pad, int dim,
                                                       float* __restrict__ qnorm, float* __restrict__ tnorm,
                                                       uint2* __restrict__ Q8, uint2* __restrict__ T8, int* __restrict__ seeds,
                                                       int t_wide)
{
    const int sub = threadIdx.x & 15, grp = threadIdx.x >> 4;
    const int qblocks = nq_pad / 64;
    const bool is_t = static_cast<int>(blockIdx.x) >= qblocks;
    const uint8_t* x = is_t ? T : Q;
    const int n = is_t ? nt : nq;
    uint2* x8 = is_t ? T8 : Q8;
    const int row0 = (is_t ? blockIdx.x - qblocks : blockIdx.x) * 64;
    const int c0 = 8 * sub;
    unsigned ld[4][2];
#pragma unroll
    for (int it = 0; it < 4; ++it) {
        const int row = row0 + it * 16 + grp;
        const uint8_t* p = x + static_cast<size_t>(row < n ? row : n - 1) * dim;
#pragma unroll
        for (int e = 0; e < 2; ++e) {
            const int c = c0 + 4 * e < dim ? c0 + 4 * e : dim - 4;
            ld[it][e] = *reinterpret_cast<const unsigned*>(p + c);
        }
    }
#pragma unroll
    for (int it = 0; it < 4; ++it) {
        const int row = row0 + it * 16 + grp;
        const bool live = row < n;
        unsigned w[2];
        int si = 0;
#pragma unroll
        for (int e = 0; e < 2; ++e) {
            w[e] = (live && c0 + 4 * e < dim) ? (ld[it][e] ^ 0x80808080u) : 0u;
            si = __builtin_amdgcn_sdot4(static_cast<int>(w[e]), static_cast<int>(w[e]), si, false);
        }
#pragma unroll
        for (int o = 8; o > 0; o >>= 1) si += __shfl_xor(si, o, 16);
        x8[static_cast<size_t>(row) * ((is_t && t_wide) ? U8_WIDE_ROW16 * 2 : U8_DP / 8) + sub] = uint2{w[0], w[1]};
        if (sub == 0) {
            if (is_t) {
                seeds[seed_pos(row)] = live ? -(si >> 1) : U8_PAD_SEED;
                if (t_wide) reinterpret_cast<int*>(T8)[u8_wide_seed_index(row)] = live ? -(si >> 1) : U8_PAD_SEED;
                if (live) tnorm[row] = static_cast<float>(si);
            } else if (live) {
                qnorm[row] = static_cast<float>(si);
            }
        }
    }
}

__global__ __launch_bounds__(256) void knn_u8_widen(const uint8_t* __restrict__ x, size_t n, float* __restrict__ y)
{
    for (size_t i = static_cast<size_t>(blockIdx.x) * 256 + threadIdx.x; i < n; i += static_cast<size_t>(gridDim.x) * 256)
        y[i] = static_cast<float>(x[i]);
}

__device__ __forceinline__ int half_exp_ceil(float norm2)
{
    int e;
    (void)__builtin_frexpf(norm2, &e);
    return (e + 1) >> 1;
}

__device__ __forceinline__ int train_half_exp(unsigned long long s0, unsigned epoch)
{
    const float tmax = static_cast<unsigned>(s0 >> 32) == epoch ? __uint_as_float(static_cast<unsigned>(s0)) : 0.f;
    return tmax > 0.f ? half_exp_ceil(tmax) : 10;
}

struct QueryScale {
    float sq;
    float unscale;
    float qc[3];
    bool unranked;
};

__device__ __forceinline__ QueryScale query_scale(int ht, float qnorm2)
{
    QueryScale g;
    const int hq = qnorm2 > 0.f ? half_exp_ceil(qnorm2) : ht;
    const int j = ht - hq;
    g.unranked = j < -3;
    const int jc = j < -3 ? -3 : (j > 7 ? 7 : j);
    g.sq = __builtin_ldexpf(1.f, 10 - ht + jc);
    g.unscale = __builtin_ldexpf(1.f, 2 * ht - 20 - jc);
    g.qc[0] = -__builtin_ldexpf(1.f, 8 + jc);
    g.qc[1] = -__builtin_ldexpf(1.f, 1 + jc);
    g.qc[2] = -__builtin_ldexpf(1.f, jc - 5);
    return g;
}

__global__ void knn_gen_off(unsigned long long* __restrict__ stats, unsigned epoch)
{
    if (threadIdx.x == 0) atomicMax(&stats[3], (static_cast<unsigned long long>(epoch) << 32) | 1ull);
}

template <int DP, bool ALIGNED>
__global__ __launch_bounds__(256) void knn_l2_prep16g(const float* __restrict__ Q, int nq, int nq_pad,
                                                      const float* __restrict__ T, int nt, int nt_pad, int dim,
                                                      const float* __restrict__ qnorm, const float* __restrict__ tnorm,
                                                      _Float16* __restrict__ Qh, _Float16* __restrict__ Th,
                                                      const unsigned long long* __restrict__ stats, unsigned epoch)
{
    typedef F16Rows<DP> G;
    constexpr int NCB = G::NCB;
    const unsigned long long s1 = stats[1];
    const bool flagged = static_cast<unsigned>(s1 >> 32) == epoch;
    if (!(flagged && (s1 & 2ull))) return;
    if (s1 & 1ull) return;
    const int ht = train_half_exp(stats[0], epoch);
    const float st = __builtin_ldexpf(1.f, 10 - ht);
    const int sub = threadIdx.x & 15, grp = threadIdx.x >> 4;
    const int qblocks = nq_pad / 64;
    const bool is_t = static_cast<int>(blockIdx.x) >= qblocks;
    const float* x = is_t ? T : Q;
    const int n = is_t ? nt : nq;
    _Float16* xh = is_t ? Th : Qh;
    const int row0 = (is_t ? blockIdx.x - qblocks : blockIdx.x) * 64;
    const int c0 = 8 * sub;
    Row8<ALIGNED> ld[4][NCB];
    float nrm[4];
#pragma unroll
    for (int it = 0; it < 4; ++it) {
        const int row = row0 + it * 16 + grp;
        const int rr = row < n ? row : n - 1;
        const float* p = x + static_cast<size_t>(rr) * dim;
#pragma unroll
        for (int cb = 0; cb < NCB; ++cb) ld[it][cb].load(p, 128 * cb + c0, dim);
        nrm[it] = (is_t ? tnorm : qnorm)[rr];
    }
#pragma unroll
    for (int it = 0; it < 4; ++it) {
        const int row = row0 + it * 16 + grp;
        const bool live = row < n;
        QueryScale qs = query_scale(ht, nrm[it]);
        const float sc = is_t ? st : qs.sq;
        const bool zero = !live || (!is_t && qs.unranked);
#pragma unroll
        for (int cb = 0; cb < NCB; ++cb) {
            float v[8];
            ld[it][cb].get(128 * cb + c0, dim, !zero, v);
            f16x8 hv;
#pragma unroll
            for (int e = 0; e < 8; ++e) hv[e] = static_cast<_Float16>(v[e] * sc);
            *reinterpret_cast<f16x8*>(xh + static_cast<size_t>(row) * G::ROWH + 128 * cb + c0) = hv;
        }
        if (sub == 0) {
            f16x8 e0 = {0, 0, 0, 0, 0, 0, 0, 0};
            const f16x8 e1 = {0, 0, 0, 0, 0, 0, 0, 0};
            if (is_t) {
                if (live) {
                    const float z = __builtin_rintf(nrm[it] * st * st * 16.f);
                    const unsigned tn = z < 16777216.f ? static_cast<unsigned>(z) : 16777215u;
                    e0[0] = static_cast<_Float16>(static_cast<float>(tn >> 13));
                    e0[1] = static_cast<_Float16>(static_cast<float>((tn >> 6) & 127u));
                    e0[2] = static_cast<_Float16>(static_cast<float>(tn & 63u));
                } else {
                    e0[0] = static_cast<_Float16>(60000.f);
                    e0[1] = static_cast<_Float16>(60000.f);
                }
            } else if (live && qs.unranked) {
                e0[0] = static_cast<_Float16>(__builtin_nanf(""));
            } else {
                e0[0] = static_cast<_Float16>(qs.qc[0]);
                e0[1] = static_cast<_Float16>(qs.qc[1]);
                e0[2] = static_cast<_Float16>(qs.qc[2]);
            }
            *reinterpret_cast<f16x8*>(xh + static_cast<size_t>(row) * G::ROWH + DP) = e0;
            *reinterpret_cast<f16x8*>(xh + static_cast<size_t>(row) * G::ROWH + DP + 8) = e1;
        }
    }
}

template <int DP, bool ALIGNED>
__global__ __launch_bounds__(256) void knn_l2_prep16u(const float* __restrict__ Q, int nq, int nq_pad,
                                                      const float* __restrict__ T, int nt, int nt_pad, int dim,
                                                      float* __restrict__ qnorm, float* __restrict__ tnorm,
                                                      _Float16* __restrict__ Qh, _Float16* __restrict__ Th,
                                                      unsigned long long* __restrict__ stats, unsigned epoch)
{
    typedef F16Rows<DP> G;
    constexpr int NCB = G::NCB;
    constexpr float BOUND2 = 1.0009765625f;
    __shared__ unsigned wbad[4];
    const int ht = half_exp_ceil(BOUND2);
    const float st = __builtin_ldexpf(1.f, 10 - ht);
    const int sub = threadIdx.x & 15, grp = threadIdx.x >> 4;
    const int qblocks = nq_pad / 64;
    const bool is_t = static_cast<int>(blockIdx.x) >= qblocks;
    const float* x = is_t ? T : Q;
    const int n = is_t ? nt : nq;
// ... 913 lines not shown
    if (k == 1)
        hipLaunchKernelGGL(knn_l2_exact<1>, grid, dim3(256), 0, ctx->stream, dq, dt, nq, nt, dim, k, dout);
    else if (k == 2)
        hipLaunchKernelGGL(knn_l2_exact<2>, grid, dim3(256), 0, ctx->stream, dq, dt, nq, nt, dim, k, dout);
    else
        hipLaunchKernelGGL(knn_l2_exact<4>, grid, dim3(256), 0, ctx->stream, dq, dt, nq, nt, dim, k, dout);
    PM_HIP_CHECK(hipGetLastError());
    return PM_OK;
}


int kf_prepare(pm_ctx* ctx, int nq, KnnFuse& fz, int queries_per_tile = 32)
{
    const int tiles = (nq + queries_per_tile - 1) / queries_per_tile;
    if (tiles > ctx->kf_cap) {
        PM_HIP_CHECK(hipStreamSynchronize(ctx->stream));
        if (ctx->kf_tile) PM_HIP_CHECK(hipFree(ctx->kf_tile));
        ctx->kf_tile = nullptr;
        ctx->kf_cap = 0;
        const int cap = tiles < 4096 ? 4096 : tiles + tiles / 2;
        PM_HIP_CHECK(hipMalloc(reinterpret_cast<void**>(&ctx->kf_tile), static_cast<size_t>(cap) * 12));
        PM_HIP_CHECK(hipMemsetAsync(ctx->kf_tile, 0, static_cast<size_t>(cap) * 12, ctx->stream));
        ctx->kf_cap = cap;
        ctx->kf_epoch = 0;
    }
    if (++ctx->kf_epoch >= (1u << 24)) {
        PM_HIP_CHECK(hipMemsetAsync(ctx->kf_tile, 0, static_cast<size_t>(ctx->kf_cap) * 12, ctx->stream));
        ctx->kf_epoch = 1;
    }
    fz.tile = ctx->kf_tile;
    fz.tilecnt = reinterpret_cast<unsigned*>(ctx->kf_tile + ctx->kf_cap);
    fz.err = reinterpret_cast<unsigned*>(ctx->knn_stats) + 12;
    fz.epoch = ctx->kf_epoch;
    return PM_OK;
}

int knn_l2_enqueue(pm_ctx* ctx, const float* dq, int nq, const float* dt, int nt, int dim, int k, int flags, pm_match* dout,
                   KnnFuse* fuse, const uint8_t* uq = nullptr, const uint8_t* ut = nullptr)
{
    const bool u8in = uq != nullptr;
    if (u8in) {
        const bool al = ((reinterpret_cast<uintptr_t>(uq) | reinterpret_cast<uintptr_t>(ut)) & 3) == 0;
        if (!(k <= 4 && (dim % 4) == 0 && dim <= 128 && nt >= 1 && al)) return 2;
        flags = PM_KNN_HINT_U8;
    }

    const bool aligned16 = u8in || ((reinterpret_cast<uintptr_t>(dq) | reinterpret_cast<uintptr_t>(dt)) & 15) == 0;
    const bool vec = (dim % 4) == 0 && aligned16;
    const bool narrow = vec && dim <= 128;
    const bool wide16 = !narrow && !(flags & PM_KNN_FORCE_F32) && ctx->opts[PM_OPT_KNN_WIDE] != 1;
    const bool fast = !(flags & PM_KNN_FORCE_EXACT) && (k <= 2 || (k <= 4 && ctx->opts[PM_OPT_KNN_WIDE] != 1)) && dim <= 256 &&
                      nt >= 1 && (narrow || wide16) && (dim >= 4 || !vec);
    if (!fast) {
        if (u8in) return 2;
        const int rx = run_exact(ctx, dq, nq, dt, nt, dim, k, dout);
        return rx == PM_OK && fuse ? 1 : rx;
    }
    int route = (flags & PM_KNN_FORCE_F32) ? ROUTE_F32 : ((flags & PM_KNN_HINT_U8) && narrow) ? ROUTE_U8_HINT :
                (flags & (PM_KNN_HINT_INTEGER | PM_KNN_HINT_U8)) ? ROUTE_F16_HINT : ROUTE_AUTO;
    const int dp16 = dim <= 128 ? 128 : 256;
    const bool unit_hint = (flags & PM_KNN_HINT_UNIT_NORM) && route == ROUTE_AUTO;
    const bool gen32 = route == ROUTE_AUTO && !unit_hint && ctx->opts[PM_OPT_KNN_GENERAL_F16] == 1 && narrow;
    const bool want32 = route == ROUTE_F32 || gen32, want16 = route != ROUTE_F32;

    constexpr int TT = TT32;
    KnnGeom g32{}, g16{};
    int splits32 = 1, splits16 = 1, lid_bits32 = 3, lid_bits16 = 4;
    {
        const int nqb = (nq + QB - 1) / QB;
        const int ntiles = (nt + TT - 1) / TT;
        int splits = (2 * ctx->n_cu + nqb - 1) / nqb;
        if (splits < (ntiles + 31) / 32) splits = (ntiles + 31) / 32;
        if (splits > ntiles) splits = ntiles;
        if (splits > 64) splits = 64;
        if (splits < 1) splits = 1;
        g32.tiles_per_split = (ntiles + splits - 1) / splits;
        splits32 = (ntiles + g32.tiles_per_split - 1) / g32.tiles_per_split;
        g32.slots = splits32 * KNN_C;
        g32.rows_per_tile = TT;
        while ((1 << lid_bits32) < g32.tiles_per_split * (TT / 8) * 2) ++lid_bits32;
        g32.lid_mask = (1u << lid_bits32) - 1u;
        g32.eps_coef = static_cast<float>((6.0 * dim + 32.0) * 5.9604644775390625e-8 * 1.001);
        g32.embed_coef = static_cast<float>(static_cast<double>(1u << lid_bits32) * 1.1920928955078125e-7 * 1.01);
    }
    const bool u8_default_group = ctx->opts[PM_OPT_KNN_U8_GROUP] != 1 && ctx->opts[PM_OPT_KNN_U8_GROUP] != 3;
    const bool u8_asked = ((flags & PM_KNN_HINT_U8) || u8in) && !(flags & PM_KNN_FORCE_F32);
    int u8_form = (u8_asked && u8_default_group) ? ctx->opts[PM_OPT_KNN_RING] : 1;
    int ws_splits = 0;
    if (u8_form == 6) {
        const int ntl = (nt + H_TT - 1) / H_TT, nqb128 = (nq + H_QB - 1) / H_QB * 2;
        int sp = (8 * ctx->n_cu + nqb128 - 1) / nqb128;
        if (sp < (ntl + 15) / 16) sp = (ntl + 15) / 16;
        if (sp > 64) sp = 64;
        if (sp > ntl) sp = ntl;
        if (sp < 1) sp = 1;
        const int tps = (ntl + sp - 1) / sp;
        const bool fits = (static_cast<long long>(nt) + 3 * H_TT) * (U8_WIDE_ROW16 * 16) < 0x7FFFFFFFLL;
        if (tps >= 8 && tps <= 16 && fits) ws_splits = sp; else u8_form = 1;
    }
    if (u8_form == 5 && (static_cast<long long>(nt) + 3 * H_TT) * (U8_WIDE_ROW16 * 16) >= 0x7FFFFFFFLL) u8_form = 1;
    const int qb_wg = u8_form >= 4 ? 128 : (u8_form >= 2 && ctx->opts[PM_OPT_KNN_F16_WAVES] == 3) ? 512 : H_QB;
    const int q_unit = qb_wg > H_QB ? qb_wg : H_QB;
    const int nq_pad = (nq + q_unit - 1) / q_unit * q_unit, nt_pad = (nt + H_TT - 1) / H_TT * H_TT;
    {
        const int nqb = nq_pad / qb_wg;
        const int ntiles = nt_pad / H_TT;
        const int wg_per_cu = ctx->opts[PM_OPT_KNN_WG_PER_CU] == 2 ? 2 : 1;
        int splits = ws_splits ? ws_splits : (wg_per_cu * ctx->n_cu + nqb - 1) / nqb;
        if (splits < (ntiles + 15) / 16) splits = (ntiles + 15) / 16;
        if (splits > ntiles) splits = ntiles;
        if (splits > 64) splits = 64;
        if (splits < 1) splits = 1;
        g16.tiles_per_split = (ntiles + splits - 1) / splits;
        splits16 = (ntiles + g16.tiles_per_split - 1) / g16.tiles_per_split;
        g16.slots = splits16 * KNN_C;
        g16.rows_per_tile = H_TT;
        while ((1 << lid_bits16) < g16.tiles_per_split * (H_TT / 8) * 2) ++lid_bits16;
        g16.lid_mask = (1u << lid_bits16) - 1u;
        g16.eps_coef = 0.f;
        g16.eps_coef_gen = static_cast<float>(9.765625e-4 * 1.125 + (6.0 * dim + 32.0) * 5.9604644775390625e-8 * 1.001);
        g16.abs_gen = static_cast<float>(dim) / 4.f + 4.f;
        g16.embed_coef = static_cast<float>(static_cast<double>(1u << lid_bits16) * 1.1920928955078125e-7 * 1.01);
    }
    const int seeded_opt = ctx->opts[PM_OPT_KNN_SEEDED];
    if (route == ROUTE_U8_HINT && (lid_bits16 > U8_SHIFT || (static_cast<long long>(nt_pad) + H_TT) * U8_DP >= 0x7FFFFFFFLL ||
                                   seeded_opt == 1))
    {
        if (u8in) return 2;
        route = ROUTE_F16_HINT;
    }
    const int u8_group = ctx->opts[PM_OPT_KNN_U8_GROUP] == 1 ? 4 : (ctx->opts[PM_OPT_KNN_U8_GROUP] == 3 ? 16 : 8);
    const bool u8_int_refine = !(ctx->opts[PM_OPT_KNN_U8_REFINE] == 1 && u8_group == 4);
    const bool f16s = route == ROUTE_F16_HINT && seeded_opt == 2 && narrow &&
                      (static_cast<long long>(nt_pad) + H_TT) * (F16S_ROW16 * 16) < 0x7FFFFFFFLL;
    const bool u8r = route == ROUTE_U8_HINT;
    if (u8r) {
        g16.lid_mask = (1u << U8_SHIFT) - 1u;
        g16.int_shift = U8_SHIFT;
        g16.embed_coef = 0.f;
    }
    if (u8in && !(route == ROUTE_U8_HINT && u8_int_refine)) return 2;
    if ((want32 && lid_bits32 > 16) || (want16 && lid_bits16 > 16)) {
        const int rx = run_exact(ctx, dq, nq, dt, nt, dim, k, dout);
        return rx == PM_OK && fuse ? 1 : rx;
    }

    const size_t c32 = want32 ? sizeof(float) * static_cast<size_t>(nq) * g32.slots : 0;
    const size_t c16 = want16 ? sizeof(float) * static_cast<size_t>(nq) * g16.slots : 0;
    const size_t rowb = u8r ? U8_DP : sizeof(_Float16) * (f16s ? H_DP : dp16 + 16);
    const size_t qh = want16 ? rowb * static_cast<size_t>(nq_pad) : 0;
    const int t_wide = (u8r && u8_form >= 5) ? 1 : 0;
    const size_t th = want16 ? (t_wide ? static_cast<size_t>(U8_WIDE_ROW16) * 16 : rowb) * static_cast<size_t>(nt_pad) : 0;
    const size_t sdb = (u8r || f16s) ? 4 * static_cast<size_t>(nt_pad + H_TT) : 0;
    const size_t pkb = fuse ? sizeof(unsigned long long) * static_cast<size_t>(nq) : 0;
    const size_t need = pm::align_up(sizeof(float) * nq, 256) + pm::align_up(sizeof(float) * nt, 256) +
                        pm::align_up(c32, 256) + pm::align_up(c16, 256) + pm::align_up(qh, 256) + pm::align_up(th, 256) +
                        pm::align_up(sdb, 256) + pm::align_up(pkb, 256) + 2048;
    int rc = pm::arena_reserve(ctx, need);
    if (rc != PM_OK) return rc;
    pm::arena_reset(ctx);
    float* qnorm = static_cast<float*>(pm::arena_take(ctx, sizeof(float) * nq));
    float* tnorm = static_cast<float*>(pm::arena_take(ctx, sizeof(float) * nt));
    float* cval32 = want32 ? static_cast<float*>(pm::arena_take(ctx, c32)) : nullptr;
    float* cval16 = want16 ? static_cast<float*>(pm::arena_take(ctx, c16)) : nullptr;
    _Float16* Qh = want16 ? static_cast<_Float16*>(pm::arena_take(ctx, qh)) : nullptr;
    _Float16* Th = want16 ? static_cast<_Float16*>(pm::arena_take(ctx, th)) : nullptr;
    void* seeds = sdb ? pm::arena_take(ctx, sdb) : nullptr;
    PM_REQUIRE(qnorm && tnorm && (!want32 || cval32) && (!want16 || (cval16 && Qh && Th)) && (!sdb || seeds), PM_E_NOMEM,
               "scratch arena too small");
    KnnFuse fz{};
    if (fuse) {
        fz = *fuse;
        fz.pk = static_cast<unsigned long long*>(pm::arena_take(ctx, pkb));
        PM_REQUIRE(fz.pk != nullptr, PM_E_NOMEM, "scratch arena too small");
        rc = kf_prepare(ctx, nq, fz, (u8r && u8_int_refine) ? 16 : 32);
        if (rc != PM_OK) return rc;
    }
    g32.cand = cval32;
    g16.cand = cval16;

    unsigned long long* stats = ctx->knn_stats;
    PM_REFUSE_CAPTURE(ctx);
    if (++ctx->knn_epoch == 0u) {
        PM_HIP_CHECK(hipMemsetAsync(stats, 0, 32, ctx->stream));
        ctx->knn_epoch = 1u;
    }
    const unsigned epoch = ctx->knn_epoch;
    unsigned* diag = nullptr;
    if (ctx->knn_diag) {
        diag = ctx->knn_diag_words;
        PM_HIP_CHECK(hipMemsetAsync(diag, 0, 12, ctx->stream));
    }
    {
        pm::ScopedKernelTime t(ctx, "knn_l2_prep");
        if (u8in)
            hipLaunchKernelGGL(knn_l2_prep8_u8, dim3(nq_pad / 64 + nt_pad / 64), dim3(256), 0, ctx->stream, uq, nq, nq_pad, ut, nt,
                               nt_pad, dim, qnorm, tnorm, reinterpret_cast<uint2*>(Qh), reinterpret_cast<uint2*>(Th),
                               static_cast<int*>(seeds), t_wide);
        else if (u8r && ctx->opts[PM_OPT_KNN_PREP_ROWS] != 1)
            hipLaunchKernelGGL(knn_l2_prep8<1>, dim3(nq_pad / 16 + nt_pad / 16), dim3(256), 0, ctx->stream, dq, nq, nq_pad, dt,
                               nt, nt_pad, dim, qnorm, tnorm, reinterpret_cast<uint2*>(Qh), reinterpret_cast<uint2*>(Th),
                               static_cast<int*>(seeds), stats, epoch, t_wide);
        else if (u8r)
            hipLaunchKernelGGL(knn_l2_prep8<4>, dim3(nq_pad / 64 + nt_pad / 64), dim3(256), 0, ctx->stream, dq, nq, nq_pad, dt,
                               nt, nt_pad, dim, qnorm, tnorm, reinterpret_cast<uint2*>(Qh), reinterpret_cast<uint2*>(Th),
                               static_cast<int*>(seeds), stats, epoch, t_wide);
        else if (f16s)
            hipLaunchKernelGGL((knn_l2_prep16<true, 128, true>), dim3(nq_pad / 64 + nt_pad / 64), dim3(256), 0, ctx->stream, dq, nq,
                               nq_pad, dt, nt, nt_pad, dim, qnorm, tnorm, Qh, Th, static_cast<float*>(seeds), stats, epoch);
        else if (unit_hint) {
#define PM_PREP16U(DP_, AL_)                                                                                              \
    hipLaunchKernelGGL((knn_l2_prep16u<DP_, AL_>), dim3(nq_pad / 64 + nt_pad / 64), dim3(256), 0, ctx->stream, dq, nq, nq_pad, dt, \
                       nt, nt_pad, dim, qnorm, tnorm, Qh, Th, stats, epoch)
            if (dp16 == 128) { if (vec) PM_PREP16U(128, true); else PM_PREP16U(128, false); }
            else { if (vec) PM_PREP16U(256, true); else PM_PREP16U(256, false); }
#undef PM_PREP16U
        }
        else if (want16) {
#define PM_PREP16(DP_, AL_)                                                                                               \
    hipLaunchKernelGGL((knn_l2_prep16<false, DP_, AL_>), dim3(nq_pad / 64 + nt_pad / 64), dim3(256), 0, ctx->stream, dq, nq,    \
                       nq_pad, dt, nt, nt_pad, dim, qnorm, tnorm, Qh, Th, nullptr, stats, epoch)
            if (dp16 == 128) { if (vec) PM_PREP16(128, true); else PM_PREP16(128, false); }
            else { if (vec) PM_PREP16(256, true); else PM_PREP16(256, false); }
#undef PM_PREP16
        }
        else
            hipLaunchKernelGGL(knn_l2_prep, dim3((nq + 63) / 64 + (nt + 63) / 64), dim3(256), 0, ctx->stream, dq, nq, dt,
                               nt, dim, qnorm, tnorm, stats, epoch);
        if (route == ROUTE_AUTO && !gen32 && !unit_hint) {
#define PM_PREP16G(DP_, AL_)                                                                                              \
    hipLaunchKernelGGL((knn_l2_prep16g<DP_, AL_>), dim3(nq_pad / 64 + nt_pad / 64), dim3(256), 0, ctx->stream, dq, nq, nq_pad, dt, \
                       nt, nt_pad, dim, qnorm, tnorm, Qh, Th, stats, epoch)
            if (dp16 == 128) { if (vec) PM_PREP16G(128, true); else PM_PREP16G(128, false); }
            else { if (vec) PM_PREP16G(256, true); else PM_PREP16G(256, false); }
#undef PM_PREP16G
        }
        else if (gen32)
            hipLaunchKernelGGL(knn_gen_off, dim3(1), dim3(64), 0, ctx->stream, stats, epoch);
        PM_HIP_CHECK(hipGetLastError());
    }
    if (u8r) {
        rc = launch_coarse_u8(ctx, Qh, Th, static_cast<const int*>(seeds), nq, nq_pad, nt, splits16, g16.tiles_per_split,
                              reinterpret_cast<int*>(cval16), g16.slots, u8_group, u8_form);
        if (rc != PM_OK) return rc;
    } else if (f16s) {
        rc = launch_coarse_f16s(ctx, Qh, Th, static_cast<const float*>(seeds), nq, nq_pad, nt, splits16, g16.tiles_per_split,
                                ~g16.lid_mask, cval16, g16.slots);
        if (rc != PM_OK) return rc;
    } else if (want16) {
        rc = launch_coarse_f16(ctx, Qh, Th, nq, nq_pad, nt, splits16, g16.tiles_per_split, ~g16.lid_mask, cval16,
                               g16.slots, stats, epoch, route == ROUTE_AUTO ? 1 : 0, dp16);
        if (rc != PM_OK) return rc;
    }
    if (want32) {
        rc = launch_coarse_f32(ctx, dq, nq, dt, nt, dim, tnorm, splits32, g32.tiles_per_split, ~g32.lid_mask, cval32,
                               g32.slots, stats, epoch, route == ROUTE_AUTO ? 1 : 0);
        if (rc != PM_OK) return rc;
    }
    if (u8r && u8_int_refine) {
        pm::ScopedKernelTime t(ctx, "knn_l2_refine");
#define PM_R8K(NS_, GROUP_, KM_, FUSE_)                                                                                    \
    hipLaunchKernelGGL((knn_l2_refine8<NS_, GROUP_, KM_, FUSE_>), dim3((nq + 15) / 16), dim3(256), 0, ctx->stream, dq, dt,  \
                       reinterpret_cast<const uint4*>(Qh), reinterpret_cast<const uint4*>(Th), qnorm, tnorm,               \
                       reinterpret_cast<const int*>(cval16), stats, epoch, diag, nq, nt, dim, k, g16.slots, g16.tiles_per_split, dout, fz, \
                       t_wide ? U8_WIDE_ROW16 : U8_ROW16)
#define PM_R8(NS_, GROUP_) do { if (fuse) PM_R8K(NS_, GROUP_, 2, true); else if (k <= 2) PM_R8K(NS_, GROUP_, 2, false); else PM_R8K(NS_, GROUP_, 4, false); } while (0)
#define PM_R8G(NS_) do { if (u8_group == 4) PM_R8(NS_, 4); else if (u8_group == 8) PM_R8(NS_, 8); else PM_R8(NS_, 16); } while (0)
        if (g16.slots <= 16) PM_R8G(1);
        else if (g16.slots <= 32) PM_R8G(2);
        else if (g16.slots <= 64) PM_R8G(4);
        else if (g16.slots <= 128) PM_R8G(8);
        else PM_R8G(16);
#undef PM_R8G
#undef PM_R8
#undef PM_R8K
        PM_HIP_CHECK(hipGetLastError());
        return PM_OK;
    }
    {
        pm::ScopedKernelTime t(ctx, "knn_l2_refine");
        const int max_slots = (want16 ? g16.slots : 0) > (want32 ? g32.slots : 0) ? g16.slots : g32.slots;
#define PM_REFINE5(VEC_, NS_, FUSE_, GEN_, KM_)                                                                      \
    hipLaunchKernelGGL((knn_l2_refine<VEC_, NS_, FUSE_, GEN_, KM_>), dim3((nq + 3) / 4), dim3(256), 0, ctx->stream, dq, dt,  \
                       qnorm, stats, epoch, diag, nq, nt, dim, k, g16, g32, route, dout, fz)
#define PM_REFINE4(VEC_, NS_, FUSE_, GEN_) do { if (k <= 2) PM_REFINE5(VEC_, NS_, FUSE_, GEN_, 2); else PM_REFINE5(VEC_, NS_, false, GEN_, 4); } while (0)
#define PM_REFINE3(NS_, FUSE_, GEN_) do { if (vec) PM_REFINE4(true, NS_, FUSE_, GEN_); else PM_REFINE4(false, NS_, FUSE_, GEN_); } while (0)
#define PM_REFINE2(NS_, FUSE_) do { if (route == ROUTE_AUTO) PM_REFINE3(NS_, FUSE_, true); else PM_REFINE3(NS_, FUSE_, false); } while (0)
#define PM_REFINE(NS_) do { if (fuse) PM_REFINE2(NS_, true); else PM_REFINE2(NS_, false); } while (0)
        if (max_slots <= 64) PM_REFINE(1);
        else if (max_slots <= 128) PM_REFINE(2);
        else if (max_slots <= 256) PM_REFINE(4);
        else PM_REFINE(8);
#undef PM_REFINE5
#undef PM_REFINE4
#undef PM_REFINE3
#undef PM_REFINE2
#undef PM_REFINE
        PM_HIP_CHECK(hipGetLastError());
    }
    return PM_OK;
}

}

extern "C" int pm_bf_knn_l2_f32_dev(pm_ctx* ctx, const float* dq, int nq, const float* dt, int nt, int dim,
                                    int k, int flags, pm_match* dout)
{
    PM_REQUIRE(ctx != nullptr, PM_E_INVALID, "ctx is null");
    PM_REQUIRE(nq >= 0 && nt >= 0 && dim >= 1 && k >= 1 && k <= PM_MAX_K, PM_E_INVALID,
               "need nq,nt >= 0, dim >= 1, 1 <= k <= PM_MAX_K");
    PM_REQUIRE(nq == 0 || (dq && dout), PM_E_INVALID, "null query/output pointer");
    PM_REQUIRE(nt == 0 || dt, PM_E_INVALID, "null train pointer");
    if (nq == 0) return PM_OK;
    PM_HIP_CHECK(hipSetDevice(ctx->device));
    return knn_l2_enqueue(ctx, dq, nq, dt, nt, dim, k, flags, dout, nullptr);
}

extern "C" int pm_bf_knn_l2_ratio_dev(pm_ctx* ctx, const float* d_q, int nq, const float* d_t, int nt, int dim, int flags,
                                      float ratio, const float* d_kp1_xy, const float* d_kp2_xy, pm_match* d_knn,
                                      pm_match* d_good, float* d_xy1, float* d_xy2, int32_t* d_n_good)
{
    PM_REQUIRE(ctx != nullptr && d_n_good != nullptr, PM_E_INVALID, "null argument");
    PM_REQUIRE(nq >= 0 && nt >= 0 && dim >= 1, PM_E_INVALID, "need nq,nt >= 0, dim >= 1");
    PM_REQUIRE(nq == 0 || (d_q && d_good), PM_E_INVALID, "null query/output pointer");
    PM_REQUIRE(nt == 0 || d_t, PM_E_INVALID, "null train pointer");
    PM_REQUIRE((d_kp1_xy == nullptr) == (d_kp2_xy == nullptr), PM_E_INVALID, "give both keypoint arrays or none");
    PM_REQUIRE(d_kp1_xy == nullptr || (d_xy1 && d_xy2), PM_E_INVALID, "null point outputs");
    PM_HIP_CHECK(hipSetDevice(ctx->device));
    if (nq == 0) {
        PM_HIP_CHECK(hipMemsetAsync(d_n_good, 0, sizeof(int32_t), ctx->stream));
        return PM_OK;
    }
    KnnFuse fz{};
    fz.ratio = ratio; fz.kp1 = d_kp1_xy; fz.kp2 = d_kp2_xy; fz.good = d_good; fz.xy1 = d_xy1; fz.xy2 = d_xy2; fz.n_out = d_n_good;
    const int fusion = ctx->opts[PM_OPT_FILTER_FUSION];
    const bool u8_hint = (flags & PM_KNN_HINT_U8) && !(flags & (PM_KNN_FORCE_F32 | PM_KNN_FORCE_EXACT));
    const bool separate = fusion == 1 || (fusion == 0 && d_knn != nullptr && !(u8_hint && u8_fused_by_default(nq)));
    int rc;
    if (!separate) {
        rc = knn_l2_enqueue(ctx, d_q, nq, d_t, nt, dim, 2, flags, d_knn, &fz);
        if (rc <= 0) return rc;
        return pm_filter_ratio_gather_dev(ctx, d_knn, nq, 2, ratio, d_kp1_xy, d_kp2_xy, d_good, d_xy1, d_xy2, d_n_good);
    }
    PM_REQUIRE(d_knn != nullptr, PM_E_INVALID, "the two-launch form needs d_knn");
    rc = knn_l2_enqueue(ctx, d_q, nq, d_t, nt, dim, 2, flags, d_knn, nullptr);
    if (rc != PM_OK) return rc;
    return pm_filter_ratio_gather_dev(ctx, d_knn, nq, 2, ratio, d_kp1_xy, d_kp2_xy, d_good, d_xy1, d_xy2, d_n_good);
}

namespace {
int u8_widened(pm_ctx* ctx, const uint8_t* dq, int nq, const uint8_t* dt, int nt, int dim, const float** fq, const float** ft)
{
    const size_t a = pm::align_up(static_cast<size_t>(nq) * dim, 64), b = static_cast<size_t>(nt) * dim;
    if ((a + b) * sizeof(float) > ctx->widen_cap) {
        PM_HIP_CHECK(hipStreamSynchronize(ctx->stream));
        if (ctx->widen) PM_HIP_CHECK(hipFree(ctx->widen));
        ctx->widen = nullptr;
        ctx->widen_cap = 0;
        const size_t cap = pm::align_up((a + b) * sizeof(float) * 5 / 4, size_t(1) << 20);
        PM_HIP_CHECK(hipMalloc(reinterpret_cast<void**>(&ctx->widen), cap));
        ctx->widen_cap = cap;
    }
    if (static_cast<size_t>(nq) * dim)
        hipLaunchKernelGGL(knn_u8_widen, dim3(256), dim3(256), 0, ctx->stream, dq, static_cast<size_t>(nq) * dim, ctx->widen);
    if (b) hipLaunchKernelGGL(knn_u8_widen, dim3(256), dim3(256), 0, ctx->stream, dt, b, ctx->widen + a);
    PM_HIP_CHECK(hipGetLastError());
    *fq = ctx->widen;
    *ft = ctx->widen + a;
    return PM_OK;
}
}

extern "C" int pm_bf_knn_l2_u8_dev(pm_ctx* ctx, const uint8_t* dq, int nq, const uint8_t* dt, int nt, int dim, int k,
                                   pm_match* dout)
{
    PM_REQUIRE(ctx != nullptr, PM_E_INVALID, "ctx is null");
    PM_REQUIRE(nq >= 0 && nt >= 0 && dim >= 1 && k >= 1 && k <= PM_MAX_K, PM_E_INVALID,
               "need nq,nt >= 0, dim >= 1, 1 <= k <= PM_MAX_K");
    PM_REQUIRE(nq == 0 || (dq && dout), PM_E_INVALID, "null query/output pointer");
    PM_REQUIRE(nt == 0 || dt, PM_E_INVALID, "null train pointer");
    if (nq == 0) return PM_OK;
    PM_HIP_CHECK(hipSetDevice(ctx->device));
    int rc = nt >= 1 ? knn_l2_enqueue(ctx, nullptr, nq, nullptr, nt, dim, k, 0, dout, nullptr, dq, dt) : 2;
    if (rc != 2) return rc;
    const float *fq = nullptr, *ft = nullptr;
    rc = u8_widened(ctx, dq, nq, dt, nt, dim, &fq, &ft);
    if (rc != PM_OK) return rc;
    return knn_l2_enqueue(ctx, fq, nq, ft, nt, dim, k, PM_KNN_HINT_INTEGER, dout, nullptr);
}

extern "C" int pm_bf_knn_l2_u8_ratio_dev(pm_ctx* ctx, const uint8_t* d_q, int nq, const uint8_t* d_t, int nt, int dim, float ratio,
                                         const float* d_kp1_xy, const float* d_kp2_xy, pm_match* d_knn, pm_match* d_good,
                                         float* d_xy1, float* d_xy2, int32_t* d_n_good)
{
    PM_REQUIRE(ctx != nullptr && d_n_good != nullptr && d_knn != nullptr, PM_E_INVALID, "null argument (the u8 form needs the record buffer)");
// ... 100 lines not shown
```

points_matching_amd/csrc/knn_shared.hpp:

```cpp
#pragma once
#include "pm_common.hpp"

namespace pm_knn {

typedef float f32x16 __attribute__((ext_vector_type(16)));
typedef float f32x4 __attribute__((ext_vector_type(4)));
typedef _Float16 f16x8 __attribute__((ext_vector_type(8)));
typedef int i32x4 __attribute__((ext_vector_type(4)));
typedef int i32x16 __attribute__((ext_vector_type(16)));

constexpr int KNN_C = 4;
constexpr int QB = 128;
constexpr int TT32 = 64;
constexpr float KNN_BIG = 3.0e38f;

constexpr int H_DP = 128;
constexpr int H_ROW = H_DP + 16;
constexpr int H_LDS_ROW = H_ROW + 8;
constexpr int H_NCH = H_ROW / 16;
constexpr int H_TT = 128;
constexpr int H_QB = 256;
constexpr float H_MAXABS = 361.f;
constexpr int H_ROW16 = H_ROW / 8;
constexpr int H_LDS_ROW16 = H_LDS_ROW / 8;

constexpr int I8_BITS = 256;
constexpr int I8_NCH = 8;
constexpr int I8_ROW16 = 16;
constexpr int I8_LDS_ROW16 = 17;
constexpr int I8_GROUP_ROWS = 8;
constexpr int I8_SHIFT = 16;
constexpr int I8_EMPTY = static_cast<int>(0x80000000u);

constexpr int U8_DP = 128;
constexpr int U8_NCH = 4;
constexpr int U8_ROW16 = 8;
constexpr int U8_LDS_ROW16 = 9;
constexpr int U8_SHIFT = 9;
constexpr int U8_PAD_SEED = -(1 << 22);
constexpr int F16S_NCH = 8;
constexpr int F16S_ROW16 = 16;
constexpr int F16S_LDS_ROW16 = 17;
constexpr int SEED_TILE_BYTES = H_TT * 4;

__host__ __device__ inline int seed_pos(int row)
{
    const int i = row & 31;
    return (row & ~31) + 16 * ((i >> 2) & 1) + (i & 3) + 4 * (i >> 3);
}

constexpr int U8_WIDE_ROW16 = 9;
__host__ __device__ inline size_t u8_wide_seed_index(int row)
{
    const int p = seed_pos(row) - (row & ~31);
    return (static_cast<size_t>(row & ~31) + (p >> 2)) * (U8_WIDE_ROW16 * 4) + U8_ROW16 * 4 + (p & 3);
}

int launch_coarse_u8(pm_ctx* ctx, const void* Q8, const void* T8, const int* seeds, int nq, int nq_pad, int nt, int splits,
                     int tiles_per_split, int* cval, int slots, int group_rows, int form);
int launch_coarse_f16s(pm_ctx* ctx, const _Float16* Qh, const _Float16* Th, const float* seeds, int nq, int nq_pad, int nt,
                       int splits, int tiles_per_split, unsigned keep_mask, float* cval, int slots);

int launch_coarse_f32(pm_ctx* ctx, const float* dq, int nq, const float* dt, int nt, int dim, const float* tnorm,
                      int splits, int tiles_per_split, unsigned keep_mask, float* cval, int slots,
                      const unsigned long long* stats, unsigned epoch, int only_if_ineligible);
int launch_coarse_f16(pm_ctx* ctx, const _Float16* Qh, const _Float16* Th, int nq, int nq_pad, int nt, int splits,
                      int tiles_per_split, unsigned keep_mask, float* cval, int slots,
                      const unsigned long long* stats, unsigned epoch, int mode, int dp = 128);

int launch_coarse_i8(pm_ctx* ctx, const void* Qe, const void* Te, int nq, int nq_pad, int nt, int splits,
                     int tiles_per_split, int* cval, int slots);

}
```

points_matching_amd/csrc/pm_capi.cpp:

```cpp
#include <cfloat>
#include <cmath>

#include "pm_common.hpp"

namespace pm {

static thread_local char g_err[512] = "";

void set_error(const char* fmt, ...)
{
    va_list ap;
    va_start(ap, fmt);
    vsnprintf(g_err, sizeof g_err, fmt, ap);
    va_end(ap);
}

int arena_reserve(pm_ctx* ctx, size_t bytes)
{
    if (bytes <= ctx->arena_cap) return PM_OK;
    PM_HIP_CHECK(hipStreamSynchronize(ctx->stream));
    if (ctx->arena) PM_HIP_CHECK(hipFree(ctx->arena));
    ctx->arena = nullptr;
    ctx->arena_cap = 0;
    size_t cap = align_up(bytes + bytes / 4, size_t(1) << 20);
// ... 48 lines not shown
}

ScopedKernelTime::~ScopedKernelTime()
{
    if (!ctx->timing || !a || !b) return;
    (void)hipEventRecord(b, ctx->stream);
    ctx->timers[name].pending.emplace_back(a, b);
}

static void drain_timers(pm_ctx* ctx)
{
    for (auto& kv : ctx->timers) {
        for (auto& ab : kv.second.pending) {
            float ms = 0.f;
            if (hipEventElapsedTime(&ms, ab.first, ab.second) == hipSuccess) {
                kv.second.total_ms += ms;
                kv.second.launches += 1;
            }
            ctx->event_pool.push_back(ab.first);
            ctx->event_pool.push_back(ab.second);
        }
        kv.second.pending.clear();
    }
}

}

using namespace pm;

extern "C" {

const char* pm_last_error(void) { return g_err; }

const char* pm_status_string(int s)
{
    switch (s) {
        case PM_OK: return "ok";
        case PM_E_INVALID: return "invalid argument";
        case PM_E_TOO_FEW: return "fewer than 8 correspondences";
        case PM_E_NO_MODEL: return "no valid model in the hypothesis range";
        case PM_E_HIP: return "HIP runtime error";
        case PM_E_NOMEM: return "out of device memory";
        case PM_E_UNSUPPORTED: return "unsupported";
        default: return "unknown status";
    }
}

int pm_version(void) { return PM_VERSION_MAJOR * 100 + PM_VERSION_MINOR; }

int pm_ctx_create(int device, pm_ctx** out)
{
    PM_REQUIRE(out != nullptr, PM_E_INVALID, "out is null");
    *out = nullptr;
    int n = 0;
    PM_HIP_CHECK(hipGetDeviceCount(&n));
    PM_REQUIRE(device >= 0 && device < n && device < PM_MAX_DEVICES, PM_E_INVALID, "no such HIP device");
    PM_HIP_CHECK(hipSetDevice(device));
    pm_ctx* c = new (std::nothrow) pm_ctx();
    PM_REQUIRE(c != nullptr, PM_E_NOMEM, "host allocation failed");
    c->device = device;
    hipDeviceProp_t prop;
    if (hipGetDeviceProperties(&prop, device) == hipSuccess) c->n_cu = prop.multiProcessorCount;
    hipError_t e = hipStreamCreateWithFlags(&c->own_stream, hipStreamNonBlocking);
    if (e != hipSuccess) {
        set_error("hipStreamCreate failed: %s", hipGetErrorString(e));
        delete c;
        return PM_E_HIP;
    }
    c->stream = c->own_stream;
    e = hipMalloc(reinterpret_cast<void**>(&c->knn_stats), 64);
    if (e == hipSuccess) e = hipMemset(c->knn_stats, 0, 64);
    if (e != hipSuccess) {
        set_error("hipMalloc failed: %s", hipGetErrorString(e));
        (void)hipStreamDestroy(c->own_stream);
        delete c;
        return PM_E_NOMEM;
    }
    c->knn_diag_words = reinterpret_cast<unsigned*>(c->knn_stats + 4);
    *out = c;
    return PM_OK;
}

int pm_ctx_destroy(pm_ctx* ctx)
{
    if (!ctx) return PM_OK;
    (void)hipSetDevice(ctx->device);
    (void)hipStreamSynchronize(ctx->stream);
    drain_timers(ctx);
    for (hipEvent_t e : ctx->event_pool) (void)hipEventDestroy(e);
    if (ctx->arena) (void)hipFree(ctx->arena);
    if (ctx->knn_stats) (void)hipFree(ctx->knn_stats);
    if (ctx->fg_counts) (void)hipFree(ctx->fg_counts);
    if (ctx->sync_words) (void)hipFree(ctx->sync_words);
    if (ctx->kf_tile) (void)hipFree(ctx->kf_tile);
    if (ctx->widen) (void)hipFree(ctx->widen);
    if (ctx->pinned) (void)hipHostFree(ctx->pinned);
    if (ctx->own_stream) (void)hipStreamDestroy(ctx->own_stream);
    delete ctx;
    return PM_OK;
}

int pm_ctx_set_stream(pm_ctx* ctx, void* hip_stream)
{
    PM_REQUIRE(ctx != nullptr, PM_E_INVALID, "ctx is null");
    PM_HIP_CHECK(hipStreamSynchronize(ctx->stream));
    ctx->stream = hip_stream ? static_cast<hipStream_t>(hip_stream) : ctx->own_stream;
    return PM_OK;
}

int pm_ctx_synchronize(pm_ctx* ctx)
{
    PM_REQUIRE(ctx != nullptr, PM_E_INVALID, "ctx is null");
    PM_HIP_CHECK(hipStreamSynchronize(ctx->stream));
    return PM_OK;
}

int pm_ctx_timing_enable(pm_ctx* ctx, int enable)
{
    PM_REQUIRE(ctx != nullptr, PM_E_INVALID, "ctx is null");
    ctx->timing = enable != 0;
    return PM_OK;
}

int pm_ctx_timing_reset(pm_ctx* ctx)
{
    PM_REQUIRE(ctx != nullptr, PM_E_INVALID, "ctx is null");
    PM_HIP_CHECK(hipStreamSynchronize(ctx->stream));
    drain_timers(ctx);
    for (auto& kv : ctx->timers) { kv.second.total_ms = 0.0; kv.second.launches = 0; }
    return PM_OK;
}

int pm_ctx_timing_get(pm_ctx* ctx, const char* kernel, double* mean_ms, int* launches)
{
    PM_REQUIRE(ctx != nullptr && kernel != nullptr, PM_E_INVALID, "null argument");
    PM_HIP_CHECK(hipStreamSynchronize(ctx->stream));
    drain_timers(ctx);
    auto it = ctx->timers.find(kernel);
    double ms = 0.0;
    int n = 0;
    if (it != ctx->timers.end()) {
        n = it->second.launches;
        ms = n ? it->second.total_ms / n : 0.0;
    }
    if (mean_ms) *mean_ms = ms;
    if (launches) *launches = n;
    return PM_OK;
}

int pm_ctx_set_option(pm_ctx* ctx, int option, int value)
{
    PM_REQUIRE(ctx != nullptr, PM_E_INVALID, "ctx is null");
    PM_REQUIRE(option >= 1 && option < PM_OPT_COUNT_, PM_E_INVALID, "unknown option");
    const int vmax = option == PM_OPT_RANSAC_WG_IDS ? 128 : option == PM_OPT_KNN_RING_PROLOGUE ? 8 : option == PM_OPT_KNN_RING ? 6 : (option == PM_OPT_KNN_F16_WAVES || option == PM_OPT_KNN_U8_GROUP) ? 3 : 2;
    PM_REQUIRE(value >= 0 && value <= vmax, PM_E_INVALID,
               "option value out of range (0 = automatic, 1, 2; KNN_F16_WAVES, KNN_U8_GROUP: .. 3)");
    ctx->opts[option] = value;
    return PM_OK;
}

int pm_ctx_get_option(pm_ctx* ctx, int option, int* value)
{
    PM_REQUIRE(ctx != nullptr && value != nullptr, PM_E_INVALID, "null argument");
    PM_REQUIRE(option >= 1 && option < PM_OPT_COUNT_, PM_E_INVALID, "unknown option");
    *value = ctx->opts[option];
    return PM_OK;
}

int pm_ctx_knn_diag_enable(pm_ctx* ctx, int enable)
{
    PM_REQUIRE(ctx != nullptr, PM_E_INVALID, "ctx is null");
    ctx->knn_diag = enable != 0;
    return PM_OK;
}

int pm_ctx_filter_fusion_status(pm_ctx* ctx, int* gave_up)
{
    PM_REQUIRE(ctx != nullptr && gave_up != nullptr, PM_E_INVALID, "null argument");
    unsigned w = 0;
    PM_HIP_CHECK(hipStreamSynchronize(ctx->stream));
    PM_HIP_CHECK(hipMemcpy(&w, reinterpret_cast<const char*>(ctx->knn_stats) + 48, sizeof w, hipMemcpyDeviceToHost));
    *gave_up = (ctx->kf_epoch != 0u && w == ctx->kf_epoch) ? 1 : 0;
    return PM_OK;
}

int pm_ctx_knn_stats(pm_ctx* ctx, int* rescans, int* nonfinite)
{
    PM_REQUIRE(ctx != nullptr, PM_E_INVALID, "ctx is null");
    unsigned h[2] = {0, 0};
    PM_HIP_CHECK(hipStreamSynchronize(ctx->stream));
    PM_HIP_CHECK(hipMemcpy(h, ctx->knn_diag_words, sizeof h, hipMemcpyDeviceToHost));
    if (rescans) *rescans = static_cast<int>(h[0]);
    if (nonfinite) *nonfinite = static_cast<int>(h[1]);
    return PM_OK;
}

int pm_ctx_knn_route(pm_ctx* ctx, int* route)
{
    PM_REQUIRE(ctx != nullptr && route != nullptr, PM_E_INVALID, "null argument");
    unsigned h = 0;
    PM_HIP_CHECK(hipStreamSynchronize(ctx->stream));
    PM_HIP_CHECK(hipMemcpy(&h, ctx->knn_diag_words + 2, sizeof h, hipMemcpyDeviceToHost));
    *route = static_cast<int>(h);
    return PM_OK;
}


int pm_filter_midpoint(const pm_match* m, int n, double* min_out, double* max_out,
                       pm_match* out, int* n_out)
{
    PM_REQUIRE(n >= 0 && (n == 0 || (m && out)) && n_out, PM_E_INVALID, "bad argument");
    double lo = 1, hi = 0;
    for (int i = 0; i < n; ++i) {
        const double d = m[i].distance;
        if (lo > d) lo = d;
        if (hi < d) hi = d;
    }
    const double cut = lo + (hi - lo) / 2;
    int kept = 0;
    for (int i = 0; i < n; ++i)
        if (static_cast<double>(m[i].distance) < cut) out[kept++] = m[i];
    if (min_out) *min_out = lo;
    if (max_out) *max_out = hi;
    *n_out = kept;
    return PM_OK;
}

int pm_filter_ratio(const pm_match* knn, int nq, int k, float ratio, pm_match* out, int* n_out)
{
    PM_REQUIRE(nq >= 0 && k >= 2 && (nq == 0 || (knn && out)) && n_out, PM_E_INVALID,
               "bad argument (ratio test needs k >= 2)");
    int kept = 0;
    for (int i = 0; i < nq; ++i) {
        const pm_match& best = knn[static_cast<size_t>(i) * k];
        const pm_match& second = knn[static_cast<size_t>(i) * k + 1];
        if (best.trainIdx < 0 || second.trainIdx < 0) continue;
        const float rhs = ratio * second.distance;
        if (best.distance < rhs) out[kept++] = best;
    }
    *n_out = kept;
    return PM_OK;
}


int pm_match_indices(const pm_match* m, int n, int32_t* query_idx, int32_t* train_idx)
{
    PM_REQUIRE(n >= 0 && (n == 0 || (m && query_idx && train_idx)), PM_E_INVALID, "bad argument");
    for (int i = 0; i < n; ++i) {
        query_idx[i] = m[i].queryIdx;
        train_idx[i] = m[i].trainIdx;
    }
    return PM_OK;
}

int pm_gather_points(const float* kp_xy, int n_kp, const int32_t* idx, int n, float* out_xy)
{
    PM_REQUIRE(n >= 0 && n_kp >= 0 && (n == 0 || (kp_xy && idx && out_xy)), PM_E_INVALID,
               "bad argument");
    for (int i = 0; i < n; ++i) {
        const int32_t j = idx[i];
        PM_REQUIRE(j >= 0 && j < n_kp, PM_E_INVALID, "keypoint index out of range");
        out_xy[2 * i] = kp_xy[2 * static_cast<size_t>(j)];
        out_xy[2 * i + 1] = kp_xy[2 * static_cast<size_t>(j) + 1];
    }
    return PM_OK;
}

long pm_format_match_list(const pm_match* m, int n, char* buf, size_t cap)
{
    if (n < 0 || (n > 0 && !m)) return -1;
    std::string s = "Good Matches are:\n";
    char line[128];
    for (int i = 0; i < n; ++i) {
        snprintf(line, sizeof line, "-- Good Match [%d] Keypoint 1: %d  -- Keypoint 2: %d  \n", i,
                 m[i].queryIdx, m[i].trainIdx);
        s += line;
    }
    if (buf && cap) {
        size_t w = s.size() < cap - 1 ? s.size() : cap - 1;
        memcpy(buf, s.data(), w);
        buf[w] = 0;
    }
    return static_cast<long>(s.size());
}


int pm_epipolar_residuals(const float* xy1, const float* xy2, int n, const double F[9],
                          int transposed, double* r, double* mean_abs)
{
    PM_REQUIRE(n >= 0 && F && (n == 0 || (xy1 && xy2)), PM_E_INVALID, "bad argument");
    const float* pa = transposed ? xy1 : xy2;
    const float* pb = transposed ? xy2 : xy1;
    double acc = 0.0;
    for (int i = 0; i < n; ++i) {
        const double xa = pa[2 * i], ya = pa[2 * i + 1];
        const double xb = pb[2 * i], yb = pb[2 * i + 1];
        double v[3];
        for (int j = 0; j < 3; ++j) {
            double t = xa * F[j] + ya * F[3 + j];
            v[j] = t + F[6 + j];
        }
        double t = v[0] * xb + v[1] * yb;
        const double res = t + v[2];
        if (r) r[i] = res;
        acc += std::fabs(res);
    }
    if (mean_abs) *mean_abs = acc / n;
    return PM_OK;
}
// ... 65 lines not shown
```

Measured before the change: 2227 billion.

## Add optional super-tile staging and fragment-ordered query copy to u8 coarse kernel

Adds a template parameter S that stages 2 or 4 train tiles per LDS-DMA round in the seeded u8 rows288 kernel, so fewer barriers and issue rounds run per tile. This is selected through a new KNN_SUPERTILE option that defaults to 1. The prep kernels also write a second query copy in B-fragment order, and the u8 two-buffer form now reads that copy so each lane loads its fragment contiguously. In exchange this costs extra LDS per workgroup when S>1, an extra query buffer and extra global writes during prep.

```diff
diff --git a/include/pm.h b/include/pm.h
--- a/include/pm.h
+++ b/include/pm.h
@@ -61,7 +61,8 @@
     PM_OPT_RANSAC_FORM    = 17,
     PM_OPT_RANSAC_WG_IDS  = 18,
     PM_OPT_HAMMING_REFINE = 19,
-    PM_OPT_COUNT_         = 20
+    PM_OPT_KNN_SUPERTILE  = 20,
+    PM_OPT_COUNT_         = 21
 };
 int  pm_ctx_set_option(pm_ctx* ctx, int option, int value);
 int  pm_ctx_get_option(pm_ctx* ctx, int option, int* value);
diff --git a/points_matching_amd/api.py b/points_matching_amd/api.py
--- a/points_matching_amd/api.py
+++ b/points_matching_amd/api.py
@@ -106,6 +106,7 @@
 PM_OPT_RANSAC_FORM = 17
 PM_OPT_RANSAC_WG_IDS = 18
 PM_OPT_HAMMING_REFINE = 19
+PM_OPT_KNN_SUPERTILE = 20
 
 
 _lib = None
diff --git a/points_matching_amd/csrc/knn_coarse.hip b/points_matching_amd/csrc/knn_coarse.hip
--- a/points_matching_amd/csrc/knn_coarse.hip
+++ b/points_matching_amd/csrc/knn_coarse.hip
@@ -28,10 +28,10 @@
                                    cval, slots, nullptr, 0u, 0);
 }
 
-int launch_coarse_u8(pm_ctx* ctx, const void* Q8, const void* T8, const int* seeds, int nq, int nq_pad, int nt, int splits,
-                     int tiles_per_split, int* cval, int slots, int group_rows, int form)
+int launch_coarse_u8(pm_ctx* ctx, const void* Q8, const void* Qf, const void* T8, const int* seeds, int nq, int nq_pad, int nt,
+                     int splits, int tiles_per_split, int* cval, int slots, int group_rows, int form)
 {
-    return coarse_u8_dispatch<AblNone>(ctx, Q8, T8, seeds, nq, nq_pad, nt, splits, tiles_per_split, cval, slots, group_rows, form);
+    return coarse_u8_dispatch<AblNone>(ctx, Q8, Qf, T8, seeds, nq, nq_pad, nt, splits, tiles_per_split, cval, slots, group_rows, form);
 }
 
 int launch_coarse_f16s(pm_ctx* ctx, const _Float16* Qh, const _Float16* Th, const float* seeds, int nq, int nq_pad, int nt,
diff --git a/points_matching_amd/csrc/knn_coarse_kernels.hpp b/points_matching_amd/csrc/knn_coarse_kernels.hpp
--- a/points_matching_amd/csrc/knn_coarse_kernels.hpp
+++ b/points_matching_amd/csrc/knn_coarse_kernels.hpp
@@ -542,12 +542,14 @@
     }
 }
 
-template <typename R, int NQB, bool DMA, int GR, typename ABL>
+template <typename R, int NQB, bool DMA, int GR, int S, typename ABL>
 __global__ __launch_bounds__(H_QB / (32 * NQB) * 64 * GR, (R::NCH > 9 ? (NQB == 2 ? 1 : 2) : (NQB == 2 ? 2 : 4))) void knn_mfma_rows288(
     const uint4* __restrict__ Qh, const uint4* __restrict__ Th, const uint4* __restrict__ seeds_g, int nq, int nt,
     int tiles_per_split, unsigned par, typename R::list* __restrict__ cand_val, int slots,
     const unsigned long long* __restrict__ stats, unsigned epoch, int mode)
 {
+    static_assert(S == 1 || ((S == 2 || S == 4) && GR == 1 && DMA && R::SEEDED), "super-tiles: the seeded LDS-DMA form, one row group");
+    ABL::stamp(0);
     typedef typename R::frag frag;
     typedef typename R::acc acc;
     typedef typename R::list list;
@@ -562,7 +564,7 @@
     extern __shared__ __attribute__((aligned(16))) uint4 hsm[];
     static_assert(!R::SEEDED || DMA, "the seeded routes stage by LDS-DMA only");
     constexpr int TILE_SLOTS = H_TT * R::LDS_ROW16;
-    uint4* const ssm = hsm + 2 * TILE_SLOTS;
+    uint4* const ssm = hsm + 2 * S * TILE_SLOTS;
     const int tid = threadIdx.x, lane = tid & 63, wave = tid >> 6;
     const int r = lane & 31, h = lane >> 5;
     const int gw = wave % WPG, grp = wave / WPG;
@@ -577,15 +579,33 @@
         const_cast<uint4*>(Th), 0, ntiles * (H_TT * R::ROW16 * 16), 0x00020000);
     const __amdgpu_buffer_rsrc_t s_rsrc = __builtin_amdgcn_make_buffer_rsrc(
         const_cast<uint4*>(R::SEEDED ? seeds_g : Th), 0, (ntiles + 1) * SEED_TILE_BYTES, 0x00020000);
-    auto seed_issue = [&](int tile, int buf) {
+    auto seed_issue = [&](int tile, int buf, int i) {
         typedef __attribute__((address_space(3))) void* lptr_t;
-        if (R::SEEDED && wave == THREADS / 64 - 1)
+        if (R::SEEDED && wave == THREADS / 64 - 1 - i)
             __builtin_amdgcn_raw_ptr_buffer_load_lds(s_rsrc, (lptr_t)(ssm + 64 * buf), 16, lane * 16, tile * SEED_TILE_BYTES, 0, 0);
     };
+    int tile1 = tile0 + tiles_per_split;
+    if (tile1 > ntiles) tile1 = ntiles;
+    const int ntl = tile1 - tile0;
+    static_assert(S <= THREADS / 64, "one wave per seed piece of a super-tile");
+    auto super_issue = [&](int u, int b) {
+#pragma unroll
+        for (int i = 0; i < S; ++i) {
+            if constexpr (S == 1) {
+                const int t = tile0 + u < ntiles ? tile0 + u : (tile0 + u - 1 < ntiles ? tile0 + u - 1 : ntiles - 1);
+                dma.issue(t_rsrc, t, hsm, b, wave);
+                seed_issue(t, b, 0);
+            } else if (S * u + i < ntl) {
+                dma.issue(t_rsrc, tile0 + S * u + i, hsm, b * S + i, wave);
+                seed_issue(tile0 + S * u + i, b * S + i, i);
+            }
+        }
+    };
+    ABL::stamp(18);
     if (DMA) {
         dma.init(lane, wave);
-        dma.issue(t_rsrc, tile0 < ntiles ? tile0 : ntiles - 1, hsm, 0, wave);
-        seed_issue(tile0 < ntiles ? tile0 : ntiles - 1, 0);
+        super_issue(0, 0);
+        ABL::stamp(19);
     } else {
         st.load(Th, tile0 < ntiles ? tile0 : ntiles - 1, tid);
     }
@@ -593,8 +613,13 @@
 #pragma unroll
     for (int qb = 0; qb < NQB; ++qb)
 #pragma unroll
-        for (int c = 0; c < R::NCH; ++c)
-            qf[qb][c] = *reinterpret_cast<const frag*>(Qh + static_cast<size_t>(qbase + 32 * qb + r) * R::ROW16 + 2 * c + h);
+        for (int c = 0; c < R::NCH; ++c) {
+            if constexpr (R::SEEDED && R::NCH == U8_NCH)
+                qf[qb][c] = *reinterpret_cast<const frag*>(Qh + (static_cast<size_t>((qbase >> 5) + qb) * R::NCH + c) * 64 + lane);
+            else
+                qf[qb][c] = *reinterpret_cast<const frag*>(Qh + static_cast<size_t>(qbase + 32 * qb + r) * R::ROW16 + 2 * c + h);
+        }
+    ABL::stamp(1);
 #pragma unroll
     for (int qb = 0; qb < NQB; ++qb)
 #pragma unroll
@@ -605,8 +630,6 @@
             qf[qb][c] = __builtin_bit_cast(frag, t);
         }
 
-    int tile1 = tile0 + tiles_per_split;
-    if (tile1 > ntiles) tile1 = ntiles;
     list cl[NQB];
 #pragma unroll
     for (int qb = 0; qb < NQB; ++qb) cl[qb] = R::empty();
@@ -614,29 +637,37 @@
     if (tile0 < tile1) {
         if (!DMA) st.store(hsm, 0, tid);
         __syncthreads();
+        ABL::stamp(2);
         acc A[NQB], B[NQB];
-        for (int tix = 0; tix < tile1 - tile0; ++tix) {
-            const int buf = tix & 1;
-            const uint4* tb = hsm + (buf * H_TT + r) * R::LDS_ROW16 + h;
+        for (int u = 0; u < (ntl + S - 1) / S; ++u) {
+            const int buf = u & 1;
             constexpr unsigned G = R::GPB;
-            const unsigned lb = static_cast<unsigned>(tix) * (4u * G);
             if constexpr (!ABL::no_stage) {
-                if (DMA) {
-                    dma.issue(t_rsrc, tile0 + tix + 1 < ntiles ? tile0 + tix + 1 : tile0 + tix, hsm, buf ^ 1, wave);
-                    seed_issue(tile0 + tix + 1 < ntiles ? tile0 + tix + 1 : tile0 + tix, buf ^ 1);
-                } else st.load(Th, tile0 + tix + 1 < ntiles ? tile0 + tix + 1 : tile0 + tix, tid);
+                if (DMA) super_issue(u + 1, buf ^ 1);
+                else st.load(Th, tile0 + u + 1 < ntiles ? tile0 + u + 1 : tile0 + u, tid);
             }
-            const uint4* sb = ssm + 64 * buf + 4 * h;
             if constexpr (GR == 1) {
-                if (tix == 0) h_block<R, NQB, false, ABL>(tb, sb, qf, A, A, 0u, par, cl);
-                else h_block<R, NQB, true, ABL>(tb, sb, qf, A, B, lb - G, par, cl);
-                h_block<R, NQB, true, ABL>(tb + 32 * R::LDS_ROW16, sb + 8, qf, B, A, lb, par, cl);
-                h_block<R, NQB, true, ABL>(tb + 64 * R::LDS_ROW16, sb + 16, qf, A, B, lb + G, par, cl);
-                if constexpr (!ABL::no_stage) {
-                    if (!DMA) st.store(hsm, buf ^ 1, tid);
+#pragma unroll
+                for (int i = 0; i < S; ++i) {
+                    const int tix = S * u + i;
+                    if (S > 1 && tix >= ntl) break;
+                    const uint4* tb = hsm + ((buf * S + i) * H_TT + r) * R::LDS_ROW16 + h;
+                    const uint4* sb = ssm + 64 * (buf * S + i) + 4 * h;
+                    const unsigned lb = static_cast<unsigned>(tix) * (4u * G);
+                    if (tix == 0) h_block<R, NQB, false, ABL>(tb, sb, qf, A, A, 0u, par, cl);
+                    else h_block<R, NQB, true, ABL>(tb, sb, qf, A, B, lb - G, par, cl);
+                    h_block<R, NQB, true, ABL>(tb + 32 * R::LDS_ROW16, sb + 8, qf, B, A, lb, par, cl);
+                    h_block<R, NQB, true, ABL>(tb + 64 * R::LDS_ROW16, sb + 16, qf, A, B, lb + G, par, cl);
+                    if constexpr (!ABL::no_stage) {
+                        if (!DMA) st.store(hsm, buf ^ 1, tid);
+                    }
+                    h_block<R, NQB, true, ABL>(tb + 96 * R::LDS_ROW16, sb + 24, qf, B, A, lb + 2u * G, par, cl);
                 }
-                h_block<R, NQB, true, ABL>(tb + 96 * R::LDS_ROW16, sb + 24, qf, B, A, lb + 2u * G, par, cl);
             } else {
+                const int tix = u;
+                const uint4* tb = hsm + (buf * H_TT + r) * R::LDS_ROW16 + h;
+                const uint4* sb = ssm + 64 * buf + 4 * h;
+                const unsigned lb = static_cast<unsigned>(tix) * (4u * G);
                 const uint4* tg = tb + grp * 64 * R::LDS_ROW16;
                 const uint4* sg = sb + 16 * grp;
                 const unsigned gb = lb + 2u * static_cast<unsigned>(grp) * G;
@@ -648,6 +679,7 @@
                 h_block<R, NQB, true, ABL>(tg + 32 * R::LDS_ROW16, sg + 8, qf, B, A, gb, par, cl);
             }
             tile_barrier<ABL>();
+            if (u < 13) ABL::stamp(3 + u);
         }
         const unsigned lb = static_cast<unsigned>(tile1 - tile0 - 1) * (4u * R::GPB) +
                             (GR == 1 ? 3u : 2u * static_cast<unsigned>(grp) + 1u) * R::GPB;
@@ -656,6 +688,7 @@
 #pragma unroll
             for (int g = 0; g < R::GPB; ++g) R::select(B[qb], par, (lb + static_cast<unsigned>(g)) << 1, cl[qb], g);
     }
+    ABL::stamp(16);
     if constexpr (GR == 2) {
         list* xs = reinterpret_cast<list*>(hsm);
 #pragma unroll
@@ -685,6 +718,7 @@
             if (q < nq) cand_val[(static_cast<size_t>(q) * slots + (wg.split * 2 + h) * KNN_C) / KNN_C] = cl[qb];
         }
     }
+    ABL::stamp(17);
 }
 
 template <int N>
@@ -914,24 +948,36 @@
 template <typename R, typename ABL>
 int launch_rows288(pm_ctx* ctx, const char* name, const void* Qh, const void* Th, const void* seeds, int nq, int nq_pad, int nt,
                    int splits, int tiles_per_split, unsigned par, void* cval, int slots, const unsigned long long* stats,
-                   unsigned epoch, int mode)
-{
-    const size_t lds = sizeof(uint4) * (2 * H_TT * R::LDS_ROW16 + (R::SEEDED ? 2 * 64 : 0));
+                   unsigned epoch, int mode, int st = 1)
+{
+    constexpr bool SUPER = std::is_same<R, RouteU8T<2>>::value;
+    PM_REQUIRE(st == 1 || (SUPER && (st == 2 || st == 4)), PM_E_INVALID, "super-tiles exist for the u8 route's 8-row groups only");
+    auto lds_of = [](int s_) { return sizeof(uint4) * s_ * (2 * H_TT * R::LDS_ROW16 + (R::SEEDED ? 2 * 64 : 0)); };
+    static_assert(!SUPER || 4 * sizeof(uint4) * (2 * H_TT * R::LDS_ROW16 + 2 * 64) <= 160 * 1024, "S = 4 exceeds the CU's LDS");
     const int nqb_opt = ctx->opts[PM_OPT_KNN_F16_WAVES];
     const int nqb = nqb_opt ? nqb_opt : (tiles_per_split <= 8 ? 1 : 2);
+    if (nqb == 3) st = 1;
+    const size_t lds = lds_of(st);
+    if constexpr (SUPER) {
+        if (st == 2) name = "knn_l2_mfma_u8_s2";
+        if (st == 4) name = "knn_l2_mfma_u8_s4";
+    }
     static bool attr_done_dev[PM_MAX_DEVICES] = {};
     bool& attr_done = attr_done_dev[ctx->device];
     if (!attr_done) {
-#define PM_ATTR(NQB_, DMA_, GR_)                                                                                  \
-    PM_HIP_CHECK(hipFuncSetAttribute(reinterpret_cast<const void*>(&knn_mfma_rows288<R, NQB_, DMA_, GR_, ABL>),        \
-                                     hipFuncAttributeMaxDynamicSharedMemorySize, static_cast<int>(lds)))
+#define PM_ATTR_S(NQB_, DMA_, GR_, S_)                                                                            \
+    PM_HIP_CHECK(hipFuncSetAttribute(reinterpret_cast<const void*>(&knn_mfma_rows288<R, NQB_, DMA_, GR_, S_, ABL>),    \
+                                     hipFuncAttributeMaxDynamicSharedMemorySize, static_cast<int>(lds_of(S_))))
+#define PM_ATTR(NQB_, DMA_, GR_) PM_ATTR_S(NQB_, DMA_, GR_, 1)
         PM_ATTR(1, true, 1); PM_ATTR(2, true, 1);
+        if constexpr (SUPER) { PM_ATTR_S(1, true, 1, 2); PM_ATTR_S(2, true, 1, 2); PM_ATTR_S(1, true, 1, 4); PM_ATTR_S(2, true, 1, 4); }
         if constexpr (!R::SEEDED) { PM_ATTR(1, false, 1); PM_ATTR(2, false, 1); }
         if constexpr (R::MERGE) {
             PM_ATTR(2, true, 2);
             if constexpr (!R::SEEDED) PM_ATTR(2, false, 2);
         }
 #undef PM_ATTR
+#undef PM_ATTR_S
         attr_done = true;
     }
     pm::ScopedKernelTime t(ctx, name);
@@ -941,9 +987,19 @@
     typename R::list* out = static_cast<typename R::list*>(cval);
     const bool dma = R::SEEDED || (ctx->opts[PM_OPT_KNN_STAGING] != 1 && rows288_dma_ok<R>(nt));
     PM_REQUIRE(!R::SEEDED || rows288_dma_ok<R>(nt), PM_E_UNSUPPORTED, "train set too large for the seeded coarse routes");
+#define PM_GOS(NQB_, DMA_, GR_, S_, THREADS_)                                                                      \
+    hipLaunchKernelGGL((knn_mfma_rows288<R, NQB_, DMA_, GR_, S_, ABL>), dim3(nq_pad / H_QB, splits), dim3(THREADS_), lds, \
+                       ctx->stream, q4, t4, s4, nq, nt, tiles_per_split, par, out, slots, stats, epoch, mode)
 #define PM_GO(NQB_, DMA_, GR_, THREADS_)                                                                           \
-    hipLaunchKernelGGL((knn_mfma_rows288<R, NQB_, DMA_, GR_, ABL>), dim3(nq_pad / H_QB, splits), dim3(THREADS_), lds,  \
-                       ctx->stream, q4, t4, s4, nq, nt, tiles_per_split, par, out, slots, stats, epoch, mode)
+    do {                                                                                                           \
+        if constexpr (SUPER && GR_ == 1) {                                                                         \
+            if (st == 4) PM_GOS(NQB_, true, 1, 4, THREADS_);                                                       \
+            else if (st == 2) PM_GOS(NQB_, true, 1, 2, THREADS_);                                                  \
+            else PM_GOS(NQB_, true, 1, 1, THREADS_);                                                               \
+        } else {                                                                                                   \
+            PM_GOS(NQB_, DMA_, GR_, 1, THREADS_);                                                                  \
+        }                                                                                                          \
+    } while (0)
 #define PM_GO2(NQB_, GR_, THREADS_)                                                                                \
     do {                                                                                                           \
         if constexpr (R::SEEDED) { PM_GO(NQB_, true, GR_, THREADS_); }                                             \
@@ -962,6 +1018,7 @@
     else PM_GO2(1, 1, 512);
 #undef PM_GO2
 #undef PM_GO
+#undef PM_GOS
     PM_HIP_CHECK(hipGetLastError());
     return PM_OK;
 }
@@ -1323,16 +1380,19 @@
 }
 
 template <typename ABL>
-int coarse_u8_dispatch(pm_ctx* ctx, const void* Q8, const void* T8, const int* seeds, int nq, int nq_pad, int nt, int splits,
-                       int tiles_per_split, int* cval, int slots, int group_rows, int form)
+int coarse_u8_dispatch(pm_ctx* ctx, const void* Q8, const void* Qf, const void* T8, const int* seeds, int nq, int nq_pad, int nt,
+                       int splits, int tiles_per_split, int* cval, int slots, int group_rows, int form)
 {
     if (form >= 4 && group_rows == 8)
         return launch_rega<2, ABL>(ctx, "knn_l2_mfma_u8", Q8, T8, seeds, nq, nq_pad, nt, splits, tiles_per_split, cval, slots, form);
     if (form >= 2 && group_rows == 8)
         return launch_ring<RouteU8T<2>, 8, ABL>(ctx, "knn_l2_mfma_u8", Q8, T8, seeds, nq, nq_pad, nt, splits, tiles_per_split, 0u, cval, slots);
+    const int st_opt = group_rows == 8 ? ctx->opts[PM_OPT_KNN_SUPERTILE] : 0;
+    const int st = st_opt == 3 ? 4 : (st_opt == 2 ? 2 : 1);
+    PM_REQUIRE(Qf != nullptr, PM_E_INVALID, "the two-buffer u8 form reads the query copy in B-fragment order");
 #define PM_U8(GPB_)                                                                                                        \
-    launch_rows288<RouteU8T<GPB_>, ABL>(ctx, "knn_l2_mfma_u8", Q8, T8, seeds, nq, nq_pad, nt, splits, tiles_per_split, 0u, cval,   \
-                                        slots, nullptr, 0u, 0)
+    launch_rows288<RouteU8T<GPB_>, ABL>(ctx, "knn_l2_mfma_u8", Qf, T8, seeds, nq, nq_pad, nt, splits, tiles_per_split, 0u, cval,   \
+                                        slots, nullptr, 0u, 0, st)
     if (group_rows == 16) return PM_U8(1);
     if (group_rows == 8) return PM_U8(2);
     return PM_U8(4);
diff --git a/points_matching_amd/csrc/knn_l2.hip b/points_matching_amd/csrc/knn_l2.hip
--- a/points_matching_amd/csrc/knn_l2.hip
+++ b/points_matching_amd/csrc/knn_l2.hip
@@ -252,7 +252,7 @@
                                                     float* __restrict__ qnorm, float* __restrict__ tnorm,
                                                     uint2* __restrict__ Q8, uint2* __restrict__ T8,
                                                     int* __restrict__ seeds, unsigned long long* __restrict__ stats,
-                                                    unsigned epoch, int t_wide)
+                                                    unsigned epoch, int t_wide, uint2* __restrict__ Qf)
 {
     __shared__ unsigned wbad[4];
     const int sub = threadIdx.x & 15, grp = threadIdx.x >> 4;
@@ -297,6 +297,7 @@
         for (int o = 8; o > 0; o >>= 1) s += __shfl_xor(s, o, 16);
         if (!okrow) bad |= 2u;
         x8[static_cast<size_t>(row) * ((is_t && t_wide) ? U8_WIDE_ROW16 * 2 : U8_DP / 8) + sub] = uint2{w[0], w[1]};
+        if (!is_t && Qf) Qf[u8_qfrag_index2(row, sub)] = uint2{w[0], w[1]};
         if (sub == 0) {
             const int si = static_cast<int>(s);
             if (is_t) {
@@ -322,7 +323,7 @@
                                                        const uint8_t* __restrict__ T, int nt, int nt_pad, int dim,
                                                        float* __restrict__ qnorm, float* __restrict__ tnorm,
                                                        uint2* __restrict__ Q8, uint2* __restrict__ T8, int* __restrict__ seeds,
-                                                       int t_wide)
+                                                       int t_wide, uint2* __restrict__ Qf)
 {
     const int sub = threadIdx.x & 15, grp = threadIdx.x >> 4;
     const int qblocks = nq_pad / 64;
@@ -357,6 +358,7 @@
 #pragma unroll
         for (int o = 8; o > 0; o >>= 1) si += __shfl_xor(si, o, 16);
         x8[static_cast<size_t>(row) * ((is_t && t_wide) ? U8_WIDE_ROW16 * 2 : U8_DP / 8) + sub] = uint2{w[0], w[1]};
+        if (!is_t && Qf) Qf[u8_qfrag_index2(row, sub)] = uint2{w[0], w[1]};
         if (sub == 0) {
             if (is_t) {
                 seeds[seed_pos(row)] = live ? -(si >> 1) : U8_PAD_SEED;
@@ -1576,10 +1578,11 @@
     const int t_wide = (u8r && u8_form >= 5) ? 1 : 0;
     const size_t th = want16 ? (t_wide ? static_cast<size_t>(U8_WIDE_ROW16) * 16 : rowb) * static_cast<size_t>(nt_pad) : 0;
     const size_t sdb = (u8r || f16s) ? 4 * static_cast<size_t>(nt_pad + H_TT) : 0;
+    const size_t qfb = (u8r && u8_form <= 1) ? qh : 0;
     const size_t pkb = fuse ? sizeof(unsigned long long) * static_cast<size_t>(nq) : 0;
     const size_t need = pm::align_up(sizeof(float) * nq, 256) + pm::align_up(sizeof(float) * nt, 256) +
                         pm::align_up(c32, 256) + pm::align_up(c16, 256) + pm::align_up(qh, 256) + pm::align_up(th, 256) +
-                        pm::align_up(sdb, 256) + pm::align_up(pkb, 256) + 2048;
+                        pm::align_up(sdb, 256) + pm::align_up(pkb, 256) + pm::align_up(qfb, 256) + 2048;
     int rc = pm::arena_reserve(ctx, need);
     if (rc != PM_OK) return rc;
     pm::arena_reset(ctx);
@@ -1590,8 +1593,9 @@
     _Float16* Qh = want16 ? static_cast<_Float16*>(pm::arena_take(ctx, qh)) : nullptr;
     _Float16* Th = want16 ? static_cast<_Float16*>(pm::arena_take(ctx, th)) : nullptr;
     void* seeds = sdb ? pm::arena_take(ctx, sdb) : nullptr;
-    PM_REQUIRE(qnorm && tnorm && (!want32 || cval32) && (!want16 || (cval16 && Qh && Th)) && (!sdb || seeds), PM_E_NOMEM,
-               "scratch arena too small");
+    void* Qf = qfb ? pm::arena_take(ctx, qfb) : nullptr;
+    PM_REQUIRE(qnorm && tnorm && (!want32 || cval32) && (!want16 || (cval16 && Qh && Th)) && (!sdb || seeds) && (!qfb || Qf),
+               PM_E_NOMEM, "scratch arena too small");
     KnnFuse fz{};
     if (fuse) {
         fz = *fuse;
@@ -1620,15 +1624,15 @@
         if (u8in)
             hipLaunchKernelGGL(knn_l2_prep8_u8, dim3(nq_pad / 64 + nt_pad / 64), dim3(256), 0, ctx->stream, uq, nq, nq_pad, ut, nt,
                                nt_pad, dim, qnorm, tnorm, reinterpret_cast<uint2*>(Qh), reinterpret_cast<uint2*>(Th),
-                               static_cast<int*>(seeds), t_wide);
+                               static_cast<int*>(seeds), t_wide, static_cast<uint2*>(Qf));
         else if (u8r && ctx->opts[PM_OPT_KNN_PREP_ROWS] != 1)
             hipLaunchKernelGGL(knn_l2_prep8<1>, dim3(nq_pad / 16 + nt_pad / 16), dim3(256), 0, ctx->stream, dq, nq, nq_pad, dt,
                                nt, nt_pad, dim, qnorm, tnorm, reinterpret_cast<uint2*>(Qh), reinterpret_cast<uint2*>(Th),
-                               static_cast<int*>(seeds), stats, epoch, t_wide);
+                               static_cast<int*>(seeds), stats, epoch, t_wide, static_cast<uint2*>(Qf));
         else if (u8r)
             hipLaunchKernelGGL(knn_l2_prep8<4>, dim3(nq_pad / 64 + nt_pad / 64), dim3(256), 0, ctx->stream, dq, nq, nq_pad, dt,
                                nt, nt_pad, dim, qnorm, tnorm, reinterpret_cast<uint2*>(Qh), reinterpret_cast<uint2*>(Th),
-                               static_cast<int*>(seeds), stats, epoch, t_wide);
+                               static_cast<int*>(seeds), stats, epoch, t_wide, static_cast<uint2*>(Qf));
         else if (f16s)
             hipLaunchKernelGGL((knn_l2_prep16<true, 128, true>), dim3(nq_pad / 64 + nt_pad / 64), dim3(256), 0, ctx->stream, dq, nq,
                                nq_pad, dt, nt, nt_pad, dim, qnorm, tnorm, Qh, Th, static_cast<float*>(seeds), stats, epoch);
@@ -1664,7 +1668,7 @@
         PM_HIP_CHECK(hipGetLastError());
     }
     if (u8r) {
-        rc = launch_coarse_u8(ctx, Qh, Th, static_cast<const int*>(seeds), nq, nq_pad, nt, splits16, g16.tiles_per_split,
+        rc = launch_coarse_u8(ctx, Qh, Qf, Th, static_cast<const int*>(seeds), nq, nq_pad, nt, splits16, g16.tiles_per_split,
                               reinterpret_cast<int*>(cval16), g16.slots, u8_group, u8_form);
         if (rc != PM_OK) return rc;
     } else if (f16s) {
diff --git a/points_matching_amd/csrc/knn_shared.hpp b/points_matching_amd/csrc/knn_shared.hpp
--- a/points_matching_amd/csrc/knn_shared.hpp
+++ b/points_matching_amd/csrc/knn_shared.hpp
@@ -49,6 +49,11 @@
     return (row & ~31) + 16 * ((i >> 2) & 1) + (i & 3) + 4 * (i >> 3);
 }
 
+__host__ __device__ inline size_t u8_qfrag_index2(int row, int sub)
+{
+    return ((static_cast<size_t>(row >> 5) * U8_NCH + (sub >> 2)) * 64 + ((sub >> 1) & 1) * 32 + (row & 31)) * 2 + (sub & 1);
+}
+
 constexpr int U8_WIDE_ROW16 = 9;
 __host__ __device__ inline size_t u8_wide_seed_index(int row)
 {
@@ -56,8 +61,8 @@
     return (static_cast<size_t>(row & ~31) + (p >> 2)) * (U8_WIDE_ROW16 * 4) + U8_ROW16 * 4 + (p & 3);
 }
 
-int launch_coarse_u8(pm_ctx* ctx, const void* Q8, const void* T8, const int* seeds, int nq, int nq_pad, int nt, int splits,
-                     int tiles_per_split, int* cval, int slots, int group_rows, int form);
+int launch_coarse_u8(pm_ctx* ctx, const void* Q8, const void* Qf, const void* T8, const int* seeds, int nq, int nq_pad, int nt,
+                     int splits, int tiles_per_split, int* cval, int slots, int group_rows, int form);
 int launch_coarse_f16s(pm_ctx* ctx, const _Float16* Qh, const _Float16* Th, const float* seeds, int nq, int nq_pad, int nt,
                        int splits, int tiles_per_split, unsigned keep_mask, float* cval, int slots);
 
diff --git a/points_matching_amd/csrc/pm_capi.cpp b/points_matching_amd/csrc/pm_capi.cpp
--- a/points_matching_amd/csrc/pm_capi.cpp
+++ b/points_matching_amd/csrc/pm_capi.cpp
@@ -224,9 +224,9 @@
 {
     PM_REQUIRE(ctx != nullptr, PM_E_INVALID, "ctx is null");
     PM_REQUIRE(option >= 1 && option < PM_OPT_COUNT_, PM_E_INVALID, "unknown option");
-    const int vmax = option == PM_OPT_RANSAC_WG_IDS ? 128 : option == PM_OPT_KNN_RING_PROLOGUE ? 8 : option == PM_OPT_KNN_RING ? 6 : (option == PM_OPT_KNN_F16_WAVES || option == PM_OPT_KNN_U8_GROUP) ? 3 : 2;
+    const int vmax = option == PM_OPT_RANSAC_WG_IDS ? 128 : option == PM_OPT_KNN_RING_PROLOGUE ? 8 : option == PM_OPT_KNN_RING ? 6 : (option == PM_OPT_KNN_F16_WAVES || option == PM_OPT_KNN_U8_GROUP || option == PM_OPT_KNN_SUPERTILE) ? 3 : 2;
     PM_REQUIRE(value >= 0 && value <= vmax, PM_E_INVALID,
-               "option value out of range (0 = automatic, 1, 2; KNN_F16_WAVES, KNN_U8_GROUP: .. 3)");
+               "option value out of range (0 = automatic, 1, 2; KNN_F16_WAVES, KNN_U8_GROUP, KNN_SUPERTILE: .. 3)");
     ctx->opts[option] = value;
     return PM_OK;
 }
```

New measurement: 2281 billion (median of 6 runs). 1.02x the previous value.
